# kaiwenShen/Do-You-Really-Need-to-Pay-2-20-Hedge-Fund-Strategy-Replication-via-Machine-Learning

Measured on AMD Instinct MI355X. Metric: seq/sec/node MTSS-WGAN-GP train (24x32 windows) at 1/2/4/8 GPUs; W-dist parity, higher is better.
Workload: dtype fp32; 1 GPU; global_batch=262144, batch_per_gpu=262144, seq_len=24, features=32, parallelism=dp1

## Files before the change

do-you-really-need-to-pay-2-20-hedge-fund-strategy-replication-via-machine-learning_amd/csrc/bindings.cpp:

```cpp
#include <torch/extension.h>
#include <torch/library.h>
#include <ATen/hip/impl/HIPGuardImplMasqueradingAsCUDA.h>
#include <ATen/hip/impl/HIPStreamMasqueradingAsCUDA.h>

#include "kernels.h"
#include "poison.h"

#include <atomic>
#include <cmath>
#include <cstdlib>
#include <cstring>

std::atomic<bool>& hfrep::poison_flag() {
  static std::atomic<bool> f{[] {
    const char* e = getenv("HFREP_POISON");
    return e && e[0] == '1';
  }()};
  return f;
}

namespace {

using at::Tensor;
using c10::optional;
// ... 229 lines not shown
  TORCH_CHECK(dzx.sizes() == gates.sizes(), "lstm_tfwd: shapes");
  const int B = gates.size(0), Tn = gates.size(1), H = gates.size(2) / 4;
  check_lstm_U(U, H);
  GUARD(dzx);
  Tensor hds = out_empty({B, Tn, H}, dzx.options());
  Tensor zds = out_empty_like(gates);
  Tensor cds = out_empty({B, Tn, H}, dzx.options());
  const bool ok = hfrep::launch_lstm_tfwd(dt_of(dzx), dzx.data_ptr(), gates.data_ptr(), cs.data_ptr(),
                                          U.data_ptr<float>(), hds.data_ptr(), zds.data_ptr(), cds.data_ptr(), B, Tn,
                                          H, (int)act, cur_stream(dzx));
  TORCH_CHECK(ok, "lstm_tfwd: hidden size ", H, " not instantiated");
  return {hds, zds, cds};
}

std::tuple<Tensor, Tensor> lstm_tbwd(optional<Tensor> dH, Tensor dHd, Tensor gates, Tensor cs, Tensor zds, Tensor cds,
                                     Tensor U, int64_t act) {
  CHECK_GPU(dHd); CHECK_GPU(gates); CHECK_GPU(cs); CHECK_GPU(zds); CHECK_GPU(cds);
  same_dt(dHd, gates); same_dt(dHd, zds); same_dt(dHd, cds);
  if (dH.has_value()) { CHECK_GPU(*dH); same_dt(*dH, dHd); }
  const int B = gates.size(0), Tn = gates.size(1), H = gates.size(2) / 4;
  check_lstm_U(U, H);
  GUARD(dHd);
  Tensor dZ = out_empty_like(gates), dZd = out_empty_like(gates);
  const bool ok = hfrep::launch_lstm_tbwd(dt_of(dHd), ptr_or_null(dH), dHd.data_ptr(), gates.data_ptr(),
                                          cs.data_ptr(), zds.data_ptr(), cds.data_ptr(), U.data_ptr<float>(),
                                          dZ.data_ptr(), dZd.data_ptr(), B, Tn, H, (int)act, cur_stream(dHd));
  TORCH_CHECK(ok, "lstm_tbwd: hidden size ", H, " not instantiated");
  return {dZ, dZd};
}

bool lstmf_supported(int64_t H, int64_t K, int64_t act) { return hfrep::lstmf_supported((int)H, (int)K, (int)act); }
bool narrowf_supported(int64_t K, int64_t N) { return hfrep::narrowf_supported((int)K, (int)N); }
int64_t set_lstmf_fwd_impl(int64_t v) { return hfrep::set_lstmf_fwd_impl((int)v); }
int64_t set_lstmf_bwd_impl(int64_t v) { return hfrep::set_lstmf_bwd_impl((int)v); }

std::tuple<Tensor, Tensor> lstmf_fwd(Tensor x, Tensor W, optional<Tensor> b, Tensor U, int64_t act, bool save) {
  CHECK_F32(x); CHECK_F32(W);
  TORCH_CHECK(x.dim() == 3, "x must be (B, T, K)");
  const int B = x.size(0), Tn = x.size(1), K = x.size(2), H = U.size(0);
  check_lstm_U(U, H);
  TORCH_CHECK(W.size(0) == K && W.size(1) == 4 * H, "W must be (K, 4H)");
  if (b.has_value()) { CHECK_F32(*b); TORCH_CHECK(b->numel() == 4 * H, "bias size"); }
  TORCH_CHECK(hfrep::lstmf_supported(H, K, (int)act), "lstmf_fwd: unsupported H/K/act");
  GUARD(x);
  Tensor hs = out_empty({B, Tn, H}, x.options());
  Tensor tape = at::empty({save ? (int64_t)hfrep::lstmf_tape_elems(B, Tn) : 0}, x.options());
  const bool ok = hfrep::launch_lstmf_fwd(x.data_ptr<float>(), W.data_ptr<float>(),
                                          b.has_value() ? b->data_ptr<float>() : nullptr, U.data_ptr<float>(),
                                          hs.data_ptr<float>(), save ? tape.data_ptr<float>() : nullptr, B, Tn, K, H,
                                          (int)act, cur_stream(x));
  TORCH_CHECK(ok, "lstmf_fwd: launch failed");
  return {hs, tape};
}

std::tuple<Tensor, Tensor> lstmf_tfwd(Tensor xd, Tensor W, Tensor U, Tensor tape, int64_t act) {
  CHECK_F32(xd); CHECK_F32(W); CHECK_F32(tape);
  TORCH_CHECK(xd.dim() == 3, "xd must be (B, T, K)");
  const int B = xd.size(0), Tn = xd.size(1), K = xd.size(2), H = U.size(0);
  check_lstm_U(U, H);
  TORCH_CHECK(W.size(0) == K && W.size(1) == 4 * H, "W must be (K, 4H)");
  TORCH_CHECK(tape.numel() == (int64_t)hfrep::lstmf_tape_elems(B, Tn), "lstmf_tfwd: tape size");
  TORCH_CHECK(hfrep::lstmf_supported(H, K, (int)act), "lstmf_tfwd: unsupported H/K/act");
  GUARD(xd);
  Tensor hds = out_empty({B, Tn, H}, xd.options());
  Tensor ttape = at::empty_like(tape);
  const bool ok = hfrep::launch_lstmf_tfwd(xd.data_ptr<float>(), W.data_ptr<float>(), U.data_ptr<float>(),
                                           tape.data_ptr<float>(), hds.data_ptr<float>(), ttape.data_ptr<float>(), B, Tn,
                                           K, H, (int)act, cur_stream(xd));
  TORCH_CHECK(ok, "lstmf_tfwd: launch failed");
  return {hds, ttape};
}

static void check_head(const optional<Tensor>& d, const optional<Tensor>& w, const Tensor& like, int64_t B, int64_t n) {
  if (d.has_value()) {
    CHECK_F32(*d);
    TORCH_CHECK(d->numel() == B && d->device() == like.device(), "head adjoint factor: B fp32 values");
  }
  if (w.has_value()) {
    CHECK_F32(*w);
    TORCH_CHECK(w->numel() == n && w->device() == like.device(), "head weight: Tn H fp32 values");
  }
}

Tensor lstmf_bwd(optional<Tensor> dH, Tensor tape, Tensor U, int64_t act, int64_t B, int64_t Tn, optional<Tensor> hd,
                 optional<Tensor> hw) {
  CHECK_F32(tape);
  const int H = U.size(0);
  check_lstm_U(U, H);
  TORCH_CHECK(tape.numel() == (int64_t)hfrep::lstmf_tape_elems(B, Tn), "lstmf_bwd: tape size");
  if (dH.has_value()) { CHECK_F32(*dH); TORCH_CHECK(dH->numel() == B * Tn * H, "lstmf_bwd: dH shape"); }
  TORCH_CHECK(hd.has_value() == hw.has_value() && !(hd.has_value() && dH.has_value()),
              "lstmf_bwd: dH or the head factors (hd, hw)");
  check_head(hd, hw, tape, B, Tn * H);
  GUARD(tape);
  Tensor dZ = out_empty({B, Tn, 4 * H}, tape.options());
  Tensor dHm;
  if (hd.has_value() && !hfrep::lstmf_head_supported()) {
    dHm = out_empty({B, Tn * H}, tape.options());
    hfrep::launch_skinny_dgrad(hfrep::DT_F32, hd->data_ptr<float>(), hw->data_ptr<float>(), dHm.data_ptr(), B,
                               (int)(Tn * H), 1, cur_stream(tape));
  }
  const bool head = hd.has_value() && !dHm.defined();
  const float* dhp = dHm.defined() ? dHm.data_ptr<float>() : dH.has_value() ? dH->data_ptr<float>() : nullptr;
  const bool ok = hfrep::launch_lstmf_bwd(dhp, tape.data_ptr<float>(), U.data_ptr<float>(), dZ.data_ptr<float>(), B, Tn,
                                          H, (int)act, cur_stream(tape), head ? hd->data_ptr<float>() : nullptr,
                                          head ? hw->data_ptr<float>() : nullptr);
  TORCH_CHECK(ok, "lstmf_bwd: unsupported H / act");
  return dZ;
}

std::tuple<Tensor, Tensor> lstmf_tbwd(optional<Tensor> dH, optional<Tensor> dHd, Tensor tape, Tensor ttape, Tensor U,
                                      int64_t act, int64_t B, int64_t Tn, optional<Tensor> hd, optional<Tensor> hdd,
                                      optional<Tensor> hw) {
  CHECK_F32(tape); CHECK_F32(ttape);
  const int H = U.size(0);
  check_lstm_U(U, H);
  TORCH_CHECK(tape.numel() == (int64_t)hfrep::lstmf_tape_elems(B, Tn) && ttape.numel() == tape.numel(), "tape size");
  for (const auto* d : {&dH, &dHd})
    if (d->has_value()) { CHECK_F32(**d); TORCH_CHECK((*d)->numel() == B * Tn * H, "lstmf_tbwd: adjoint shape"); }
  const bool head = hw.has_value();
  TORCH_CHECK(!head || (!dH.has_value() && !dHd.has_value()), "lstmf_tbwd: adjoints (dH, dHd) or head factors, not both");
  check_head(hd, hw, tape, B, Tn * H);
  check_head(hdd, {}, tape, B, Tn * H);
  GUARD(tape);
  Tensor dZ = out_empty({B, Tn, 4 * H}, tape.options()), dZd = out_empty({B, Tn, 4 * H}, tape.options());
  const bool ok = hfrep::launch_lstmf_tbwd(dH.has_value() ? dH->data_ptr<float>() : nullptr,
                                           dHd.has_value() ? dHd->data_ptr<float>() : nullptr, tape.data_ptr<float>(),
                                           ttape.data_ptr<float>(), U.data_ptr<float>(), dZ.data_ptr<float>(),
                                           dZd.data_ptr<float>(), B, Tn, H, (int)act, cur_stream(tape),
                                           head && hd.has_value() ? hd->data_ptr<float>() : nullptr,
                                           head && hdd.has_value() ? hdd->data_ptr<float>() : nullptr,
                                           head ? hw->data_ptr<float>() : nullptr);
  TORCH_CHECK(ok, "lstmf_tbwd: unsupported H / act");
  return {dZ, dZd};
}

Tensor lstmf_dgrad(Tensor dz, Tensor W, int64_t impl) {
  CHECK_F32(dz); CHECK_F32(W);
  TORCH_CHECK(dz.dim() == 2 && dz.is_contiguous() && W.dim() == 2 && W.is_contiguous() && W.size(1) == dz.size(1),
              "lstmf_dgrad: dz (M, N) and W (KO, N), contiguous");
  TORCH_CHECK(hfrep::lstmf_dgrad_supported(dz.size(1), W.size(0)), "lstmf_dgrad: N must be 400 and KO <= 112");
  GUARD(dz);
  Tensor x = out_empty({dz.size(0), W.size(0)}, dz.options());
  if (dz.size(0) == 0) return x;
  const bool ok = hfrep::launch_lstmf_dgrad(dz.data_ptr<float>(), W.data_ptr<float>(), x.data_ptr<float>(), dz.size(0),
                                            dz.size(1), W.size(0), cur_stream(dz), (int)impl);
  TORCH_CHECK(ok, "lstmf_dgrad: launch failed");
  return x;
}

bool is_fp3(const Tensor& t) { return t.scalar_type() == at::kBFloat16 && t.dim() >= 2 && t.size(-2) == 3; }

Tensor fp3_split(Tensor x, bool interleave) {
  CHECK_F32(x);
  TORCH_CHECK(x.is_contiguous() && x.dim() >= 1, "fp3_split: a contiguous fp32 tensor");
  const int64_t C = x.size(-1), M = C ? x.numel() / C : 0;
  auto sz = x.sizes().vec();
  sz.insert(sz.end() - 1, 3);
  GUARD(x);
  Tensor p = out_empty(sz, x.options().dtype(at::kBFloat16));
  hfrep::launch_fp3_split(x.data_ptr<float>(), reinterpret_cast<uint16_t*>(p.data_ptr()), M, (int)C, interleave,
                          cur_stream(x));
  return p;
}

Tensor fp3_join(Tensor p, bool interleave) {
  CHECK_GPU(p);
  TORCH_CHECK(is_fp3(p) && p.is_contiguous(), "fp3_join: contiguous bf16 planes (..., 3, C)");
  const int64_t C = p.size(-1), M = C ? p.numel() / (3 * C) : 0;
  auto sz = p.sizes().vec();
  sz.erase(sz.end() - 2);
  GUARD(p);
  Tensor x = out_empty(sz, p.options().dtype(at::kFloat));
  hfrep::launch_fp3_join(reinterpret_cast<const uint16_t*>(p.data_ptr()), x.data_ptr<float>(), M, (int)C, interleave,
                         cur_stream(p));
  return x;
}

void lstmf_wgrad_p_(Tensor x, Tensor hs, Tensor dZ, Tensor gW, Tensor gU, optional<Tensor> gb, optional<Tensor> xd,
                    optional<Tensor> hds, optional<Tensor> dZd, int64_t impl) {
  CHECK_GPU(x); CHECK_GPU(hs); CHECK_GPU(dZ);
  const int pm = (is_fp3(x) ? 1 : 0) | (is_fp3(hs) ? 2 : 0) | (is_fp3(dZ) ? 4 : 0);
  for (const Tensor* t : {&x, &hs, &dZ})
    TORCH_CHECK(t->is_contiguous() && (is_fp3(*t) ? t->dim() == 4 : (t->scalar_type() == at::kFloat && t->dim() == 3)),
                "lstmf_wgrad_p_: fp32 (B,T,C) or FP3 planes (B,T,3,C), contiguous");
  const int B = x.size(0), Tn = x.size(1), K = x.size(-1), Hd = hs.size(-1), N = dZ.size(-1);
  TORCH_CHECK(hs.size(0) == B && dZ.size(0) == B && hs.size(1) == Tn && dZ.size(1) == Tn, "lstmf_wgrad_p_: B/T");
  TORCH_CHECK(hfrep::lstmf_wgrad_supported(K, Hd, N) && (pm == 0 || K == 32 || K == 100), "lstmf_wgrad_p_: K / H / N");
  CHECK_F32(gW); CHECK_F32(gU);
  TORCH_CHECK(gW.numel() == (int64_t)K * N && gU.numel() == (int64_t)Hd * N, "lstmf_wgrad_p_: grad sizes");
// ... 449 lines not shown
  return out;
}

Tensor p2p_buffer(int64_t cap, int64_t device) {
  TORCH_CHECK(cap > 0, "p2p_buffer: cap must be positive");
  bool fine = false;
  void* p = hfrep::p2p_alloc(cap, (int)device, &fine);
  auto opts = at::TensorOptions().dtype(at::kByte).device(at::Device(at::kCUDA, (int)device));
  return torch::from_blob(p, {(int64_t)hfrep::p2p_buffer_bytes(cap)}, [](void* q) { hfrep::p2p_free(q); }, opts);
}

std::vector<int64_t> p2p_handle(Tensor buf) {
  TORCH_CHECK(buf.is_cuda() && buf.scalar_type() == at::kByte, "p2p_handle: a p2p_buffer tensor");
  uint8_t h[64];
  hfrep::p2p_ipc_handle(buf.data_ptr(), h);
  return std::vector<int64_t>(h, h + 64);
}

int64_t p2p_open(std::vector<int64_t> handle, int64_t device) {
  TORCH_CHECK(handle.size() == 64, "p2p_open: a 64-byte IPC handle");
  uint8_t h[64];
  for (int i = 0; i < 64; ++i) h[i] = (uint8_t)handle[i];
  return (int64_t)reinterpret_cast<intptr_t>(hfrep::p2p_ipc_open(h, (int)device));
}

void p2p_close(int64_t ptr) { hfrep::p2p_ipc_close(reinterpret_cast<void*>((intptr_t)ptr)); }

void p2p_allreduce_(Tensor x, Tensor buf, std::vector<int64_t> peers, int64_t rank, int64_t cap, double scale,
                    double timeout_s) {
  CHECK_F32(x);
  TORCH_CHECK(buf.is_cuda() && buf.scalar_type() == at::kByte && buf.device() == x.device(),
              "p2p_allreduce_: buf must be this device's p2p_buffer");
  const int world = (int)peers.size();
  TORCH_CHECK(world >= 1 && world <= hfrep::kP2PMaxRanks && rank >= 0 && rank < world, "p2p_allreduce_: 1 <= world <= 8");
  TORCH_CHECK(x.numel() <= cap && buf.numel() >= (int64_t)hfrep::p2p_buffer_bytes(cap), "p2p_allreduce_: x exceeds cap");
  TORCH_CHECK(peers[rank] == (int64_t)reinterpret_cast<intptr_t>(buf.data_ptr()), "p2p_allreduce_: peers[rank] must be buf");
  hfrep::P2PPeers pp{};
  for (int r = 0; r < world; ++r) pp.base[r] = reinterpret_cast<char*>((intptr_t)peers[r]);
  TORCH_CHECK(timeout_s > 0, "p2p_allreduce_: timeout_s must be positive");
  GUARD(x);
  static thread_local int s_dev = -1;
  static thread_local double s_sec = -1;
  static thread_local uint64_t s_ticks = 0;
  if (s_dev != x.get_device() || s_sec != timeout_s) {
    s_ticks = hfrep::p2p_timeout_ticks(timeout_s, x.get_device());
    s_dev = x.get_device();
    s_sec = timeout_s;
  }
  hfrep::launch_p2p_allreduce(x.data_ptr<float>(), x.numel(), pp, (int)rank, world, cap, (float)scale, s_ticks,
                              cur_stream(x));
}

int64_t p2p_error(Tensor buf) {
  TORCH_CHECK(buf.is_cuda() && buf.scalar_type() == at::kByte, "p2p_error: a p2p_buffer tensor");
  GUARD(buf);
  return hfrep::p2p_read_error(buf.data_ptr());
}

}

TORCH_LIBRARY(hfrep, m) {
  m.def("linear(Tensor x, Tensor W, Tensor? b, int act, Tensor(a!)? out=None) -> Tensor");
  m.def("linear_dgrad(Tensor dz, Tensor W) -> Tensor");
  m.def("linear_wgrad_(Tensor x, Tensor dz, Tensor(a!) gW, Tensor(b!)? gb, int shiftT=0) -> ()");
  m.def("fp3_split(Tensor x, bool interleave=False) -> Tensor");
  m.def("fp3_join(Tensor p, bool interleave=False) -> Tensor");
  m.def("lstmf_wgrad_p_(Tensor x, Tensor hs, Tensor dZ, Tensor(a!) gW, Tensor(b!) gU, Tensor(c!)? gb, Tensor? xd=None, Tensor? hds=None, Tensor? dZd=None, int impl=0) -> ()");
  m.def("lstmf_dgrad_p(Tensor dzp, Tensor W, int impl=0) -> Tensor");
  m.def("lstm_wgrad_(Tensor x, Tensor hs, Tensor dZ, Tensor(a!) gW, Tensor(b!) gU, Tensor(c!)? gb, Tensor? xd=None, Tensor? hds=None, Tensor? dZd=None, int impl=0) -> ()");
  m.def("act_fwd(Tensor x, int act) -> Tensor");
  m.def("act_bwd(Tensor dy, Tensor y, int act) -> Tensor");
  m.def("act_tangent_bwd(Tensor dyd, Tensor y, Tensor zd, int act) -> Tensor");
  m.def("lstm_fwd(Tensor zx, Tensor U, int act, bool save) -> (Tensor, Tensor, Tensor)");
  m.def("lstm_bwd(Tensor dH, Tensor gates, Tensor cs, Tensor U, int act) -> Tensor");
  m.def("lstm_tfwd(Tensor dzx, Tensor gates, Tensor cs, Tensor U, int act) -> (Tensor, Tensor, Tensor)");
  m.def("lstm_tbwd(Tensor? dH, Tensor dHd, Tensor gates, Tensor cs, Tensor zds, Tensor cds, Tensor U, int act) -> (Tensor, Tensor)");
  m.def("lstmf_supported(int H, int K, int act) -> bool", &lstmf_supported);
  m.def("narrowf_supported(int K, int N) -> bool", &narrowf_supported);
  m.def("set_lstmf_fwd_impl(int v) -> int", &set_lstmf_fwd_impl);
  m.def("set_lstmf_bwd_impl(int v) -> int", &set_lstmf_bwd_impl);
  m.def("lstmf_fwd(Tensor x, Tensor W, Tensor? b, Tensor U, int act, bool save) -> (Tensor, Tensor)");
  m.def("linear_head_cs(Tensor x, Tensor W, Tensor? b, int split, float wa, float wb, Tensor(a!) gW, Tensor(b!)? gb) -> Tensor");
  m.def("linear_head_cs_supported(int K) -> bool", &linear_head_cs_supported);
  m.def("lstmf_bwd(Tensor? dH, Tensor tape, Tensor U, int act, int B, int T, Tensor? hd=None, Tensor? hw=None) -> Tensor");
  m.def("lstmf_tbwd(Tensor? dH, Tensor? dHd, Tensor tape, Tensor ttape, Tensor U, int act, int B, int T, Tensor? hd=None, "
        "Tensor? hdd=None, Tensor? hw=None) -> (Tensor, Tensor)");
  m.def("lstmf_tfwd(Tensor xd, Tensor W, Tensor U, Tensor tape, int act) -> (Tensor, Tensor)");
  m.def("lstmf_dgrad(Tensor dz, Tensor W, int impl=0) -> Tensor");
  m.def("lstm2_fwd(Tensor x, Tensor W, Tensor? b, Tensor U, int act, bool save) -> (Tensor, Tensor)");
  m.def("lstm2_bwd(Tensor? dH, Tensor tape, Tensor U, int act, Tensor? W=None, bool need_dz=True, Tensor? head_d=None, "
        "Tensor? head_w=None) -> (Tensor, Tensor)");
  m.def("lstm2_tfwd(Tensor xd, Tensor W, Tensor U, Tensor tape, int act) -> (Tensor, Tensor)");
  m.def("lstm2_tbwd(Tensor? dH, Tensor? dHd, Tensor tape, Tensor ttape, Tensor U, int act, Tensor? W=None, "
        "Tensor? head_d=None, Tensor? head_dd=None, Tensor? head_w=None) -> (Tensor, Tensor, Tensor, Tensor)");
  m.def("set_debug_poison(bool on) -> bool", &set_debug_poison);
  m.def("layernorm_fwd(Tensor x, Tensor gamma, Tensor beta, float eps, bool save=True, float pre_lrelu=-1.0) -> "
        "(Tensor, Tensor, Tensor)");
  m.def("layernorm_bwd_(Tensor dy, Tensor xhat, Tensor rstd, Tensor gamma, Tensor(a!)? ggamma, Tensor(b!)? gbeta) -> Tensor");
  m.def("layernorm_tfwd(Tensor xd, Tensor xhat, Tensor rstd, Tensor gamma) -> Tensor");
  m.def("layernorm_tbwd_(Tensor? dy, Tensor dyd, Tensor xd, Tensor xhat, Tensor rstd, Tensor gamma, "
        "Tensor(a!) ggamma, Tensor(b!) gbeta, bool need_dx) -> (Tensor, Tensor)");
  m.def("gp_coef(Tensor g, float weight) -> (Tensor, Tensor)");
  m.def("gp_coef_pack(Tensor g, float weight, Tensor w) -> (Tensor, Tensor)");
  m.def("gp_pack(Tensor pen, float weight, Tensor w) -> Tensor");
  m.def("gan_loss(Tensor p, int split, float la, float lb, int kind) -> (Tensor, Tensor)");
  m.def("im2col_causal(Tensor x, int k, int dil) -> Tensor");
  m.def("col2im_causal(Tensor dcols, int k, int dil, int C) -> Tensor");
  m.def("interpolate(Tensor real, Tensor fake, Tensor alpha) -> Tensor");
  m.def("philox_fill_(Tensor(a!) out, int seed, Tensor(b!) ctr, int dist) -> ()");
  m.def("sample_windows(Tensor data, int batch, int seed, Tensor(a!) ctr, ScalarType out_dtype, Tensor(b!)? dst=None) -> Tensor");
  m.def("ae_fit_supported(int A, int k, int batch) -> bool", &ae_fit_supported);
  m.def("ae_fit(Tensor[] Xt, Tensor[] Xv, Tensor[] order, Tensor(a!)[] We, Tensor(b!)[] Wd, Tensor(c!)[] mWe, "
        "Tensor(d!)[] vWe, Tensor(e!)[] mWd, Tensor(f!)[] vWd, Tensor(g!)[] step, Tensor(h!)[] m_cache, int[] patience, "
        "float lr, float b1, float b2, float eps, int batch, bool bf16) -> (Tensor, Tensor)");
  m.def("rmsprop_(Tensor(a!) p, Tensor g, Tensor(b!) ms, float lr, float rho, float eps, float clip, float gscale) -> ()");
  m.def("adam_(Tensor(a!) p, Tensor g, Tensor(b!) m, Tensor(c!) v, Tensor step, float lr, float b1, float b2, float eps, float clip, float gscale) -> ()");
  m.def("nadam_(Tensor(a!) p, Tensor g, Tensor(b!) m, Tensor(c!) v, Tensor step, Tensor m_cache, float lr, float b1, float b2, float eps, float gscale) -> ()");
  m.def("step_advance_(Tensor(a!) step, Tensor(b!)? m_cache, float b1) -> ()");
  m.def("clip_(Tensor(a!) p, float c) -> ()");
  m.def("wdist_sorted(Tensor x, Tensor ref_sorted) -> Tensor");
  m.def("p2p_buffer(int cap, int device) -> Tensor", &p2p_buffer);
  m.def("p2p_handle(Tensor buf) -> int[]");
  m.def("p2p_open(int[] handle, int device) -> int", &p2p_open);
  m.def("p2p_close(int ptr) -> ()", &p2p_close);
  m.def("p2p_allreduce_(Tensor(a!) x, Tensor buf, int[] peers, int rank, int cap, float scale, float timeout_s) -> ()");
  m.def("p2p_error(Tensor buf) -> int");
}

TORCH_LIBRARY_IMPL(hfrep, CUDA, m) {
  m.impl("linear", &linear);
  m.impl("p2p_handle", &p2p_handle);
  m.impl("p2p_allreduce_", &p2p_allreduce_);
  m.impl("p2p_error", &p2p_error);
  m.impl("linear_dgrad", &linear_dgrad);
  m.impl("linear_wgrad_", &linear_wgrad_);
  m.impl("lstm_wgrad_", &lstm_wgrad_);
  m.impl("act_fwd", &act_fwd);
  m.impl("act_bwd", &act_bwd);
  m.impl("act_tangent_bwd", &act_tangent_bwd);
  m.impl("lstm_fwd", &lstm_fwd);
  m.impl("lstmf_fwd", &lstmf_fwd);
  m.impl("lstmf_tfwd", &lstmf_tfwd);
  m.impl("linear_head_cs", &linear_head_cs);
  m.impl("lstmf_bwd", &lstmf_bwd);
  m.impl("lstmf_tbwd", &lstmf_tbwd);
  m.impl("lstmf_dgrad", &lstmf_dgrad);
  m.impl("fp3_split", &fp3_split);
  m.impl("fp3_join", &fp3_join);
  m.impl("lstmf_wgrad_p_", &lstmf_wgrad_p_);
  m.impl("lstmf_dgrad_p", &lstmf_dgrad_p);
  m.impl("lstm_bwd", &lstm_bwd);
  m.impl("lstm_tfwd", &lstm_tfwd);
  m.impl("lstm_tbwd", &lstm_tbwd);
  m.impl("lstm2_fwd", &lstm2_fwd);
  m.impl("lstm2_bwd", &lstm2_bwd);
  m.impl("lstm2_tfwd", &lstm2_tfwd);
  m.impl("lstm2_tbwd", &lstm2_tbwd);
  m.impl("layernorm_fwd", &layernorm_fwd);
  m.impl("layernorm_bwd_", &layernorm_bwd_);
  m.impl("layernorm_tfwd", &layernorm_tfwd);
  m.impl("layernorm_tbwd_", &layernorm_tbwd_);
  m.impl("gp_coef", &gp_coef);
  m.impl("gp_coef_pack", &gp_coef_pack);
  m.impl("gp_pack", &gp_pack);
  m.impl("gan_loss", &gan_loss);
  m.impl("im2col_causal", &im2col_causal);
  m.impl("col2im_causal", &col2im_causal);
  m.impl("interpolate", &interpolate);
  m.impl("philox_fill_", &philox_fill_);
  m.impl("sample_windows", &sample_windows);
  m.impl("ae_fit", &ae_fit);
  m.impl("rmsprop_", &rmsprop_);
  m.impl("adam_", &adam_);
  m.impl("nadam_", &nadam_);
  m.impl("step_advance_", &step_advance_);
  m.impl("clip_", &clip_);
  m.impl("wdist_sorted", &wdist_sorted);
}
```

do-you-really-need-to-pay-2-20-hedge-fund-strategy-replication-via-machine-learning_amd/csrc/kernels.h:

```cpp
#pragma once
#include <hip/hip_runtime.h>
#include <stdint.h>

namespace hfrep {

enum DType : int { DT_F32 = 0, DT_BF16 = 1 };

bool launch_lstm_fwd(int dt, const void* zx, const float* U, void* hs, void* gates, void* cs, int B, int Tn, int H,
                     int act, hipStream_t s);
bool launch_lstm_bwd(int dt, const void* dH, const void* gates, const void* cs, const float* U, void* dZ, int B,
                     int Tn, int H, int act, hipStream_t s);
bool launch_lstm_tfwd(int dt, const void* dzx, const void* gates, const void* cs, const float* U, void* hds,
                      void* zds, void* cds, int B, int Tn, int H, int act, hipStream_t s);
bool launch_lstm_tbwd(int dt, const void* dH, const void* dHd, const void* gates, const void* cs, const void* zds,
                      const void* cds, const float* U, void* dZ, void* dZd, int B, int Tn, int H, int act,
                      hipStream_t s);

size_t lstm2_tape_elems(int B, int Tn);
bool lstm2_supported(int H, int K);
void launch_lstm2_fwd(const void* x, const float* W, const float* b, const float* U, void* hs, void* tape, int B, int Tn,
                      int K, int H, int act, hipStream_t s);
void launch_lstm2_tfwd(const void* xd, const float* W, const float* U, const void* tape, void* hds, void* ttape, int B,
                       int Tn, int K, int H, int act, hipStream_t s);
void launch_lstm2_bwd(const void* dH, const void* tape, const float* U, void* dZ, const float* W, void* dX, int K,
                      int B, int Tn, int H, int act, hipStream_t s, const void* head_d = nullptr,
                      const float* hw = nullptr);
void launch_lstm2_tbwd(const void* dH, const void* dHd, const void* tape, const void* ttape, const float* U, void* dZ,
                       void* dZd, const float* W, void* dX, void* dXd, int K, int B, int Tn, int H, int act,
                       hipStream_t s, const void* head_d = nullptr, const void* head_dd = nullptr,
                       const float* hw = nullptr);

bool lstmf_supported(int H, int K, int act);
size_t lstmf_tape_elems(int B, int Tn);
bool launch_lstmf_fwd(const float* x, const float* W, const float* b, const float* U, float* hs, float* tape, int B,
                      int Tn, int K, int H, int act, hipStream_t s);
bool launch_lstmf_tfwd(const float* xd, const float* W, const float* U, const float* tape, float* hds, float* ttape,
                       int B, int Tn, int K, int H, int act, hipStream_t s);
bool launch_lstmf_bwd(const float* dH, const float* tape, const float* U, float* dZ, int B, int Tn, int H, int act,
                      hipStream_t s, const float* hd = nullptr, const float* hw = nullptr);
bool lstmf_head_supported();
bool launch_lstmf_tbwd(const float* dH, const float* dHd, const float* tape, const float* ttape, const float* U, float* dZ,
                       float* dZd, int B, int Tn, int H, int act, hipStream_t s, const float* hd = nullptr,
                       const float* hdd = nullptr, const float* hw = nullptr);
bool lstmf_wgrad_supported(int K, int H, int N);
size_t lstmf_wgrad_workspace_floats(int M, int K, int impl = 0);
bool launch_lstmf_wgrad(const void* X, const void* Hs, const void* D, const void* Xd, const void* Hds, const void* Dd,
                        float* gW, float* gU, float* gb, int M, int K, int Tn, float* ws, hipStream_t s, int impl = 0,
                        int pm = 0);
bool lstmf_dgrad_supported(int N, int KO);
int set_lstmf_fwd_impl(int v);
int set_lstmf_bwd_impl(int v);
bool launch_lstmf_dgrad(const void* D, const float* W, float* X, int M, int N, int KO, hipStream_t s, int impl = 0,
                        bool pd = false);
void launch_fp3_split(const float* x, uint16_t* p, int64_t M, int C, bool interleave, hipStream_t s);
void launch_fp3_join(const uint16_t* p, float* x, int64_t M, int C, bool interleave, hipStream_t s);

bool ae_fit_supported(int A, int k, int batch);
struct AeFitJob {
  const float* Xt;
  const float* Xv;
  const int* order;
  float *We, *Wd, *mWe, *vWe, *mWd, *vWd, *step, *m_cache;
  double* hist;
  int* nep;
  int nt, nv, epochs, patience, k, pad_;
};
void launch_ae_fit(bool bf16, const AeFitJob* jobs, int njobs, int batch, float lr, float b1, float b2, float eps, int A,
                   hipStream_t s);

void launch_linear(int dt, const void* A, const float* W, const float* bias, void* C, int M, int N, int K,
                   int w_trans, int act, hipStream_t s);
bool fp32_exact_mode();
size_t wgrad_workspace_floats(int M, int K, int N);
void launch_wgrad(int dt, const void* X, const void* D, float* gW, float* gb, int M, int K, int N, int shiftT,
                  float* ws, hipStream_t s);

size_t lstm_wgrad2_workspace_floats(int M, int K, int Hd, int N);
void launch_lstm_wgrad2(const void* X0, const void* H0, const void* D0, const void* X1, const void* H1, const void* D1,
                        float* gW, float* gU, float* gb, int M, int K, int Hd, int N, int Tn, float* ws, hipStream_t s);
void launch_lstm_wgrad2_reduce(const float* ws, float* gW, float* gU, float* gb, int splits, int K, int Hd, int N,
                               hipStream_t s, int Ks = 0);
void launch_linear2(const void* A, const float* W, const float* bias, void* C, int M, int N, int K, int w_trans, int act,
                    hipStream_t s);

bool lstm_wgrad3_supported(int M, int K, int Hd, int N);
size_t lstm_wgrad3_workspace_floats(int K, int Hd, int N);
bool launch_lstm_wgrad3(const void* X0, const void* H0, const void* D0, const void* X1, const void* H1, const void* D1,
                        float* gW, float* gU, float* gb, int M, int K, int Hd, int N, int Tn, float* ws, hipStream_t s);

bool skinny_supported(int K, int N);
bool narrow_supported(int K, int N);
void launch_narrow_fwd(const void* x, const float* W, const float* b, void* y, int M, int K, int N, int act,
                       hipStream_t s);
bool narrowf_supported(int K, int N);
bool widef_supported(int K, int N);
void launch_widef(const float* x, const float* B, int sk, int sn, const float* b, float* y, int M, int K, int N,
                  int act, hipStream_t s);
void launch_narrowf(const float* x, const float* B, int sk, int sn, const float* b, float* y, int M, int K, int N,
                    int act, hipStream_t s);
void launch_skinny_fwd(int dt, const void* x, const float* W, const float* b, void* y, int M, int K, int N, int act,
                       hipStream_t s);
size_t skinny_wgrad_workspace_floats(int M, int K, int N);
void launch_skinny_wgrad(int dt, const void* x, const void* d, float* gW, float* gb, int M, int K, int N, float* ws,
                         hipStream_t s);
void launch_skinny_dgrad(int dt, const void* d, const float* W, void* dx, int M, int K, int N, hipStream_t s);
bool skinny_fwd_cs_supported(int K);
size_t skinny_fwd_cs_workspace_floats(int M, int K);
void launch_skinny_fwd_cs(int dt, const void* x, const float* W, const float* b, void* y, int M, int K, int split,
                          float wa, float wb, float* gW, float* gb, float* ws, hipStream_t s);
void launch_split_reduce(const float* slab, float* a, float* b, int splits, int na, int nb, hipStream_t s);

int device_cu_count();
void launch_im2col_causal(int dt, const void* x, void* cols, int B, int Tn, int C, int k, int dil, hipStream_t s);
void launch_col2im_causal(int dt, const void* dcols, void* dx, int B, int Tn, int C, int k, int dil, hipStream_t s);
void launch_act_fwd(int dt, const void* x, void* y, int64_t n, int act, hipStream_t s);
void launch_act_bwd(int dt, const void* dy, const void* y, void* dx, int64_t n, int act, hipStream_t s);
void launch_act_tangent_bwd(int dt, const void* dyd, const void* y, const void* zd, void* out, int64_t n, int act,
                            hipStream_t s);
void launch_layernorm_fwd(int dt, const void* x, const float* gamma, const float* beta, void* y, void* xhat,
                          float* rstd, int64_t rows, int D, float eps, float pre_alpha, hipStream_t s);
int layernorm_bwd_splits(int64_t rows);
void launch_layernorm_bwd(int dt, const void* dy, const void* xhat, const float* rstd, const float* gamma,
                          void* dx, float* ggamma, float* gbeta, float* ws, int64_t rows, int D, hipStream_t s);
// ... 48 lines not shown
```

do-you-really-need-to-pay-2-20-hedge-fund-strategy-replication-via-machine-learning_amd/csrc/lstm_f32.hip:

```cpp
#include "common.h"
#include "kernels.h"

#include <atomic>
#include <cstdlib>
#include <mutex>
#include <type_traits>
#include <set>
#include <stdexcept>

namespace hfrep {

namespace {

typedef __amdgpu_buffer_rsrc_t rsrc_t;
typedef int v4i_t __attribute__((ext_vector_type(4)));
constexpr int kOOB = 0x7fff0000;

__device__ __forceinline__ rsrc_t make_rsrc(const void* p, int bytes) {
  return __builtin_amdgcn_make_buffer_rsrc(const_cast<void*>(p), 0, bytes, 0x00020000);
}
__device__ __forceinline__ rsrc_t ftile_rsrc(const float* base, int row0, int B, int Tn, int W) {
  row0 = __builtin_amdgcn_readfirstlane(row0);
  const int nr = base ? max(0, min(32, B - row0)) : 0;
  return make_rsrc(base + (nr ? (size_t)row0 * Tn * W : 0), nr * Tn * W * 4);
// ... 633 lines not shown
          const int sd = tt * FH * 4 + 16 * n;
          tg[n] = __builtin_bit_cast(f32x4, __builtin_amdgcn_raw_buffer_load_b128(rt, tok ? tl : kOOB, sg, 0));
          tz[n] = __builtin_bit_cast(f32x4, __builtin_amdgcn_raw_buffer_load_b128(rtt, tok ? tl : kOOB, sg, 0));
          tcp[n] = ld1(rt, (tok && tt > 0) ? tcl : kOOB, sc);
          tcdp[n] = ld1(rtt, (tok && tt > 0) ? tcl : kOOB, sc);
          if constexpr (HEAD) {
            const float wv = ld1(rhw, tok ? hvo : kOOB, sd);
            tdh[n] = hdv[m] * wv;
            tdhd[n] = hddv[m] * wv;
          } else {
            tdh[n] = ld1(rdh, tok ? vp1[m] : kOOB, sd);
            tdhd[n] = ld1(rdhd, tok ? vp1[m] : kOOB, sd);
          }
        }
      };
#pragma unroll
      for (int m = 0; m < 2; ++m)
#pragma unroll
        for (int n = 0; n < FNT; ++n) {
          const bool tok = !(w == 3 && n >= 4);
          const int oc = tcl + (Tn - 1) * FT_STEP * 4 + ftape_slot(m, n);
          acn[m][n] = 0.f;
          acdn[m][n] = 0.f;
          tc[m][n] = ld1(rt, tok ? oc : kOOB, 0);
          tcd[m][n] = ld1(rtt, tok ? oc : kOOB, 0);
        }
      load_half(std::integral_constant<int, 0>{}, Tn - 1, true);
      for (int i = tid; i < 2 * 32 * (BZ_LR + BH_LR); i += 512) zt[i] = 0.f;
      __syncthreads();
      auto half_b = [&](auto M_) {
        constexpr int m = decltype(M_)::value;
#pragma unroll
        for (int n = 0; n < FNT; ++n) {
          const bool tok = !(w == 3 && n >= 4);
          const float i_ = tg[n][0], f_ = tg[n][1], g_ = tg[n][2], o_ = tg[n][3];
          const float zdi = tz[n][0], zdf = tz[n][1], zdg = tz[n][2], zdo = tz[n][3];
          const float c = tc[m][n], cd = tcd[m][n], cp = tcp[n], cdp = tcdp[n];
          const float si = i_ * (1.f - i_), sf = f_ * (1.f - f_), so = o_ * (1.f - o_), sg = act_dy(ACT, g_);
          const float idot = si * zdi, fdot = sf * zdf, gdot = sg * zdg, odot = so * zdo;
          const float ca = act_f(ACT, c), d1 = act_dy(ACT, ca), d2 = act_d2y(ACT, ca);
          const int hi = hr + 16 * m * BH_LR + 4 * n;
          const float a_h = tdh[n] + ht[hi], a_hd = tdhd[n] + hdt[hi];
          const float a_od = a_hd * ca;
          const float a_o = a_h * ca + a_hd * d1 * cd;
          const float a_cd = acdn[m][n] + a_hd * o_ * d1;
          const float a_c = acn[m][n] + a_h * o_ * d1 + a_hd * (odot * d1 + o_ * d2 * cd);
          const float a_fd = a_cd * cp, a_id = a_cd * g_, a_gd = a_cd * i_;
          const float a_f = a_c * cp + a_cd * cdp;
          const float a_i = a_c * g_ + a_cd * gdot;
          const float a_g = a_c * i_ + a_cd * idot;
          acn[m][n] = tok ? a_c * f_ + a_cd * fdot : 0.f;
          acdn[m][n] = tok ? a_cd * f_ : 0.f;
          const float s2i = si * (1.f - 2.f * i_), s2f = sf * (1.f - 2.f * f_), s2o = so * (1.f - 2.f * o_);
          const float s2g = act_d2y(ACT, g_);
          float zd4[4], z4[4];
          zd4[0] = a_id * si; zd4[1] = a_fd * sf; zd4[2] = a_gd * sg; zd4[3] = a_od * so;
          z4[0] = a_i * si + a_id * s2i * zdi;
          z4[1] = a_f * sf + a_fd * s2f * zdf;
          z4[2] = a_g * sg + a_gd * s2g * zdg;
          z4[3] = a_o * so + a_od * s2o * zdo;
          const int zo = zw + 16 * m * BZ_LR + 4 * n;
          float* zp = tok ? zt + zo : trash;
          float* zdp = tok ? zdt + zo : trash;
#pragma unroll
          for (int k = 0; k < 4; ++k) {
            zp[k * BZ_KQ] = z4[k];
            zdp[k * BZ_KQ] = zd4[k];
          }
          tc[m][n] = cp;
          tcd[m][n] = cdp;
          if ((n + 1) % HFREP_TBWD_CELLGROUP == 0 || n == FNT - 1) __builtin_amdgcn_sched_barrier(0);
        }
      };
      using I0 = std::integral_constant<int, 0>;
      using I1 = std::integral_constant<int, 1>;
      for (int t = Tn - 1; t >= 0; --t) {
        half_b(I0{});
        __builtin_amdgcn_sched_barrier(0);
        load_half(I1{}, t, true);
        lds_barrier();
        half_b(I1{});
        __builtin_amdgcn_sched_barrier(0);
        load_half(I0{}, t > 0 ? t - 1 : 0, t > 0);
        lds_barrier();
      }
      __syncthreads();
    }
  }
}

constexpr int WF_R = 16, WF_LA = 272, WF_LD = 400;
template <int KX>
struct WFGeo {
  static constexpr int KR = KX + FH + 1;
  static constexpr int NI = (KR + 15) / 16;
  static_assert(NI <= 16 && 16 * 16 <= WF_LA, "wgrad i tiles");
  static constexpr int NX4 = WF_R * KX / 4, NH4 = WF_R * FH / 4, ND4 = WF_R * FG / 4;
  static constexpr int JX = (NX4 + 511) / 512, JH = (NH4 + 511) / 512, JD = (ND4 + 511) / 512;
};

template <int KX, int XR = KX>
__global__ void __launch_bounds__(512)
lstmf_wgrad_kernel(const float* __restrict__ X, const float* __restrict__ Hs, const float* __restrict__ D,
                   const float* __restrict__ Xd, const float* __restrict__ Hds, const float* __restrict__ Dd,
                   float* __restrict__ slab, int M, int Tn, int rows_per_wg) {
  using WG = WFGeo<KX>;
  constexpr int NI = WG::NI, KR = WG::KR;
  __shared__ __attribute__((aligned(16))) float As[2][WF_R * WF_LA];
  __shared__ __attribute__((aligned(16))) float Ds[2][WF_R * WF_LD];
  __shared__ __attribute__((aligned(16))) float trash4[4];
  const int tid = threadIdx.x, lane = tid & 63;
  const int w = __builtin_amdgcn_readfirstlane(tid >> 6);
  const int g = lane >> 4, c16 = lane & 15;
  const int mb = blockIdx.x * rows_per_wg, me = min(M, mb + rows_per_wg);
  for (int i = tid; i < 2 * WF_R * WF_LA; i += 512) (&As[0][0])[i] = 0.f;

  f32x4 acc[NI][3], accx[2];
#pragma unroll
  for (int it = 0; it < NI; ++it)
#pragma unroll
    for (int jj = 0; jj < 3; ++jj) acc[it][jj] = f32x4{0.f, 0.f, 0.f, 0.f};
  accx[0] = accx[1] = f32x4{0.f, 0.f, 0.f, 0.f};
  const int ie0 = min(2 * w, 15), ie1 = min(2 * w + 1, 15);

  f32x4 vx[WG::JX], vh[WG::JH], vd[WG::JD];
  for (int seg = 0; seg < (Xd ? 2 : 1); ++seg) {
    const float* Xs = seg ? Xd : X;
    const float* Hq = seg ? Hds : Hs;
    const float* Dq = seg ? Dd : D;
    const int hb = mb > 0 ? mb - 1 : 0, nr = me > mb ? me - mb : 0;
    const rsrc_t rx = make_rsrc(Xs + (size_t)mb * XR, nr * XR * 4);
    const rsrc_t rh = make_rsrc(Hq + (size_t)hb * FH, (nr ? me - hb : 0) * FH * 4);
    const rsrc_t rd = make_rsrc(Dq + (size_t)mb * FG, nr * FG * 4);
    auto load = [&](int m0) {
#pragma unroll
      for (int j = 0; j < WG::JX; ++j) {
        const int e = tid + 512 * j, r = e / (KX / 4), c = e - r * (KX / 4);
        const bool ok = e < WG::NX4 && m0 + r < me;
        vx[j] = ldx4<XR>(rx, ok ? ((m0 - mb + r) * XR + 4 * c) * 4 : kOOB, 0, 4 * c);
      }
#pragma unroll
      for (int j = 0; j < WG::JH; ++j) {
        const int e = tid + 512 * j, r = e / (FH / 4), c = e - r * (FH / 4);
        const int m = m0 + r;
        const bool ok = e < WG::NH4 && m < me && (m % Tn) != 0;
        vh[j] = __builtin_bit_cast(f32x4, __builtin_amdgcn_raw_buffer_load_b128(rh, ok ? ((m - 1 - hb) * FH + 4 * c) * 4 : kOOB, 0, 0));
      }
#pragma unroll
      for (int j = 0; j < WG::JD; ++j) {
        const int e = tid + 512 * j, r = e / (FG / 4), c = e - r * (FG / 4);
        const bool ok = e < WG::ND4 && m0 + r < me;
        vd[j] = __builtin_bit_cast(f32x4, __builtin_amdgcn_raw_buffer_load_b128(rd, ok ? ((m0 - mb + r) * FG + 4 * c) * 4 : kOOB, 0, 0));
      }
    };
    auto to_lds = [&](int buf) {
#pragma unroll
      for (int j = 0; j < WG::JX; ++j) {
        const int e = tid + 512 * j, r = e / (KX / 4), c = e - r * (KX / 4);
        *reinterpret_cast<f32x4*>(e < WG::NX4 ? &As[buf][r * WF_LA + 4 * c] : trash4) = vx[j];
      }
#pragma unroll
      for (int j = 0; j < WG::JH; ++j) {
        const int e = tid + 512 * j, r = e / (FH / 4), c = e - r * (FH / 4);
        *reinterpret_cast<f32x4*>(e < WG::NH4 ? &As[buf][r * WF_LA + KX + 4 * c] : trash4) = vh[j];
      }
#pragma unroll
// ... 806 lines not shown
            t6 = mma32(a0, up[ks][n][2], t6);
            t6 = mma32(a1, up[ks][n][1], t6);
            t6 = mma32(a1, up[ks][n][0], t6);
            t6 = mma32(a0, up[ks][n][1], t6);
            acc[n] = mma32(a0, up[ks][n][0], t6);
          }
          __builtin_amdgcn_sched_barrier(0);
        }
        {
          const float at = *reinterpret_cast<const __attribute__((address_space(3))) float*>(hcur + aht + 16 * m * 16);
#pragma unroll
          for (int n = 0; n < FNT; ++n) acc[n] = mma4(at, ut[n], acc[n]);
        }
#pragma unroll
        for (int n = 0; n < FNT; ++n) {
          const bool tok = !(w == 3 && n >= 4);
          const int v1 = tok ? p1 + 16 * n : kOOB;
          const f32x4 zs = acc[n];
          float hv;
          if constexpr (!TAN) {
            float y[4];
#pragma unroll
            for (int i = 0; i < 4; ++i) {
              const float s_ = zs[i] + bq[n];
              const float e = am * __builtin_amdgcn_rcpf(1.f + __builtin_amdgcn_exp2f(s_)) + bm;
              y[i] = glin ? s_ : e;
            }
            quad_transpose(y, q);
            const float cn = y[1] * cst[m][n] + y[0] * y[2];
            float ca;
            if constexpr (ACT == ACT_TANH) ca = 2.f * __builtin_amdgcn_rcpf(1.f + __builtin_amdgcn_exp2f(GSC * cn)) - 1.f;
            else if constexpr (ACT == ACT_SIGMOID) ca = __builtin_amdgcn_rcpf(1.f + __builtin_amdgcn_exp2f(GSC * cn));
            else ca = cn;
            hv = tok ? y[3] * ca : 0.f;
            cst[m][n] = cn;
            if constexpr (TAPE) {
              st4(f32x4{y[0], y[1], y[2], y[3]}, rt, tok ? tl + tb + ftape_slot(m, n) : kOOB);
              st1(cn, rt, tok ? tcl + tb + ftape_slot(m, n) : kOOB, 0);
            }
          } else {
            float zd[4] = {zs[0], zs[1], zs[2], zs[3]};
            quad_transpose(zd, q);
            const f32x4 y = pg[n];
            const float idot = y[0] * (1.f - y[0]) * zd[0], fdot = y[1] * (1.f - y[1]) * zd[1];
            const float gdot = act_dy(ACT, y[2]) * zd[2], odot = y[3] * (1.f - y[3]) * zd[3];
            const float c = pc[n];
            float cdn = fdot * cprev[m][n] + y[1] * cst[m][n] + idot * y[2] + y[0] * gdot;
            const float ca = act_f(ACT, c);
            float hd = odot * ca + y[3] * act_dy(ACT, ca) * cdn;
            if (!tok) { cdn = 0.f; hd = 0.f; }
            cst[m][n] = cdn;
            cprev[m][n] = c;
            hv = hd;
            st4(f32x4{zd[0], zd[1], zd[2], zd[3]}, rt, tok ? tl + tb + ftape_slot(m, n) : kOOB);
            st1(cdn, rt, tok ? tcl + tb + ftape_slot(m, n) : kOOB, 0);
          }
          {
            const int u = ub + 4 * n, row = 16 * m + 4 * g + q;
            const uint32_t h1 = trunc_hi(hv);
            const float r1 = hv - __builtin_bit_cast(float, h1);
            const uint32_t m1 = trunc_hi(r1);
            const uint32_t l1 = __builtin_bit_cast(uint32_t, r1 - __builtin_bit_cast(float, m1));
            const bool pl = u < 96;
            lds_char* dp = pl ? hnext + (row * FS_HR + u) * 2 : trashc;
            *reinterpret_cast<__attribute__((address_space(3))) uint16_t*>(dp) = (uint16_t)(h1 >> 16);
            *reinterpret_cast<__attribute__((address_space(3))) uint16_t*>(dp + (pl ? FS_HPL : 0)) = (uint16_t)(m1 >> 16);
            *reinterpret_cast<__attribute__((address_space(3))) uint16_t*>(dp + (pl ? 2 * FS_HPL : 0)) = (uint16_t)(l1 >> 16);
            const bool tl4 = u >= 96 && u < FH;
            lds_char* tp = tl4 ? hnext + 3 * FS_HPL + (row * 4 + (u - 96)) * 4 : trashc;
            *reinterpret_cast<__attribute__((address_space(3))) float*>(tp) = hv;
          }
          st1(hv, rh, v1, 0);
        }
      }
      xp.to_lds(xb + ((t + 1) & 1) * 32 * GX::LR, trash);
      lds_barrier();
    }
  }
}

constexpr int BS_LZ = 432;
constexpr int BS_PL = 32 * BS_LZ * 2;

template <int ACT, bool HEAD = false>
__global__ void __launch_bounds__(256, 1)
lstmf_bwds_kernel(const float* __restrict__ dH, const float* __restrict__ tape, const float* __restrict__ U,
                  float* __restrict__ dZ, int B, int Tn, const float* __restrict__ hd, const float* __restrict__ hw) {
  extern __shared__ __attribute__((aligned(16))) float fsm[];
  float* zt = fsm;
  float* ht = zt + 32 * BZ_LR;
  float* trash = ht + 32 * BH_LR;
  lds_char* trashp = (lds_char*)(trash + 4 * BZ_KQ);
  lds_char* zp = (lds_char*)(trash + 4 * BZ_KQ + 4);
  const int tid = threadIdx.x, lane = tid & 63;
  const int w = __builtin_amdgcn_readfirstlane(tid >> 6);
  const int q = lane & 3, g = lane >> 4, j4 = (lane & 15) >> 2, c16 = lane & 15;
  const int nrb = (B + 31) / 32;
  bf16x8 up[2][DS_KS][3];
#pragma unroll
  for (int e = 0; e < 2; ++e) {
    const int col = 16 * (2 * w + e) + c16;
    const bool ok = col < FH;
#pragma unroll
    for (int ks = 0; ks < DS_KS; ++ks) {
      f32x4 v[2];
#pragma unroll
      for (int j = 0; j < 8; ++j) {
        const int k = min(32 * ks + 8 * g + j, FG - 1);
        const float x = U[(ok ? col : 0) * FG + (k & 3) * FH + (k >> 2)];
        v[j >> 2][j & 3] = (ok && 32 * ks + 8 * g + j < FG) ? x : 0.f;
      }
      uint32_t p0[3][2], p1[3][2];
      split3(v[0], p0);
      split3(v[1], p1);
#pragma unroll
      for (int p = 0; p < 3; ++p) {
        up[e][ks][p] = __builtin_bit_cast(bf16x8, make_uint4(p0[p][0], p0[p][1], p1[p][0], p1[p][1]));
        if (e == 1 || ks < 8) asm volatile("" : "+a"(up[e][ks][p]));
      }
    }
  }
  const int ub = FUW * w + j4;
  const int hr = (4 * g + q) * BH_LR + ub, zw = (4 * g + q) * BZ_LR + ub;
  const int zpw = ((4 * g + q) * BS_LZ + 4 * ub) * 2;
  const int ao = (c16 * BS_LZ + 8 * g) * 2;
  const int srr = tid / 100, sch = tid - 100 * srr, sqq = sch / 25, sc = sch - 25 * sqq;
  const int slo = (srr & 1) * BZ_LR + sqq * BZ_KQ + 4 * sc;
  const int sgo = tid < 200 ? (srr * Tn * FG + sqq * FH + 4 * sc) * 4 : kOOB;
  const int tl = ftape_lane(w, lane), tcl = ftape_cell(w, lane);
  using I0 = std::integral_constant<int, 0>;
  using I1 = std::integral_constant<int, 1>;
  for (int rb = blockIdx.x; rb < nrb; rb += gridDim.x) {
    const int row0 = rb * 32;
    const rsrc_t rdh = ftile_rsrc(dH, row0, B, Tn, FH), rt = ftape_rsrc(tape, rb, nrb, Tn);
    const rsrc_t rz = ftile_rsrc(dZ, row0, B, Tn, FG);
    const int nr = min(32, B - row0);
    int vp1[2];
#pragma unroll
    for (int m = 0; m < 2; ++m) vp1[m] = ((16 * m + 4 * g + q) * Tn * FH + ub) * 4;
    float hdv[2] = {0.f, 0.f};
    const rsrc_t rhw = make_rsrc(hw, HEAD ? Tn * FH * 4 : 0);
    if constexpr (HEAD) {
#pragma unroll
      for (int m = 0; m < 2; ++m) {
        const int r = row0 + 16 * m + 4 * g + q;
        hdv[m] = r < B ? hd[r] : 0.f;
      }
    }
    const int hvo = ub * 4;
    float dc[2][FNT], tc[2][FNT];
    f32x4 tg[FNT];
    float tcp[FNT], tdh[FNT];
    const int T1 = Tn - 1;
#pragma unroll
    for (int n = 0; n < FNT; ++n) {
      const bool tok = !(w == 3 && n >= 4);
#pragma unroll
      for (int m = 0; m < 2; ++m) {
        dc[m][n] = 0.f;
        tc[m][n] = ld1(rt, tok ? tcl + T1 * FT_STEP * 4 + ftape_slot(m, n) : kOOB, 0);
      }
      bwdf_tape_load_u<HEAD>(tg[n], tcp[n], tdh[n], rt, rdh, tl, tcl, vp1[0], T1 * FT_STEP * 4 + ftape_slot(0, n),
                             max(T1 - 1, 0) * FT_STEP * 4 + ftape_slot(0, n), T1 * FH * 4 + 16 * n, tok, T1 > 0, hdv[0],
                             rhw, hvo);
    }
    for (int i = tid; i < 3 * BS_PL / 16; i += 256)
      reinterpret_cast<__attribute__((address_space(3))) u32x4_t*>(zp)[i] = u32x4_t{0, 0, 0, 0};
    for (int i = tid; i < 32 * BH_LR; i += 256) ht[i] = 0.f;
    __syncthreads();
    auto store_half = [&](auto M_, int ts) {
      constexpr int M = decltype(M_)::value;
#pragma unroll
      for (int k = 8 * M; k < 8 * M + 8; ++k) {
        const f32x4 v = *reinterpret_cast<const f32x4*>(zt + slo + 2 * k * BZ_LR);
        st16(v, rz, 2 * k + srr < nr, sgo, (2 * k * Tn + ts) * FG * 4);
      }
    };
    auto cell = [&](auto M_, int n, float hrec, int t) {
      constexpr int m = decltype(M_)::value;
      const bool tok = !(w == 3 && n >= 4);
      const float ig = tg[n][0], fg = tg[n][1], gg = tg[n][2], og = tg[n][3];
      const float dht = tdh[n] + hrec;
      const float ca = act_f(ACT, tc[m][n]);
      const float dov = dht * ca;
      const float dct = dc[m][n] + dht * og * act_dy(ACT, ca);
      dc[m][n] = tok ? dct * fg : 0.f;
      f32x4 z4;
      z4[0] = dct * gg * ig * (1.f - ig);
      z4[1] = dct * tcp[n] * fg * (1.f - fg);
      z4[2] = dct * ig * act_dy(ACT, gg);
      z4[3] = dov * og * (1.f - og);
      float* zd = tok ? zt + zw + 16 * m * BZ_LR + 4 * n : trash;
#pragma unroll
      for (int k = 0; k < 4; ++k) zd[k * BZ_KQ] = z4[k];
      uint32_t p[3][2];
      split3(z4, p);
      lds_char* pd = tok ? zp + zpw + 16 * m * BS_LZ * 2 + 32 * n : trashp;
      const int ps = tok ? BS_PL : 0;
#pragma unroll
      for (int pp = 0; pp < 3; ++pp)
        *reinterpret_cast<__attribute__((address_space(3))) u32x2_t*>(pd + pp * ps) = u32x2_t{p[pp][0], p[pp][1]};
      tc[m][n] = tcp[n];
      if constexpr (m == 0) {
        bwdf_tape_load_u<HEAD>(tg[n], tcp[n], tdh[n], rt, rdh, tl, tcl, vp1[1], t * FT_STEP * 4 + ftape_slot(1, n),
                               max(t - 1, 0) * FT_STEP * 4 + ftape_slot(1, n), t * FH * 4 + 16 * n, tok, t > 0, hdv[1],
                               rhw, hvo);
      } else {
        const int tp = t > 0 ? t - 1 : 0;
        bwdf_tape_load_u<HEAD>(tg[n], tcp[n], tdh[n], rt, rdh, tl, tcl, vp1[0], tp * FT_STEP * 4 + ftape_slot(0, n),
                               max(tp - 1, 0) * FT_STEP * 4 + ftape_slot(0, n), tp * FH * 4 + 16 * n, tok && t > 0,
                               tp > 0, hdv[0], rhw, hvo);
      }
    };
    auto phase = [&](auto MA_, int t) {
      constexpr int MA = decltype(MA_)::value;
      if constexpr (MA == 1) {
        if (t < T1) store_half(I1{}, t + 1);
      } else {
        store_half(I0{}, t);
      }
      float hv[FNT];
#pragma unroll
      for (int n = 0; n < FNT; ++n) hv[n] = ht[hr + 16 * (1 - MA) * BH_LR + 4 * n];
      __builtin_amdgcn_sched_barrier(0);
      f32x4 acc[2] = {f32x4{0.f, 0.f, 0.f, 0.f}, f32x4{0.f, 0.f, 0.f, 0.f}};
      const lds_char* ar = zp + ao + 16 * MA * BS_LZ * 2;
      bf16x8 af[2][3];
#pragma unroll
      for (int p = 0; p < 3; ++p) af[0][p] = *reinterpret_cast<const __attribute__((address_space(3))) bf16x8*>(ar + p * BS_PL);
#pragma unroll
      for (int ks = 0; ks < DS_KS; ++ks) {
        if (ks + 1 < DS_KS) {
#pragma unroll
          for (int p = 0; p < 3; ++p)
            af[(ks + 1) & 1][p] = *reinterpret_cast<const __attribute__((address_space(3))) bf16x8*>(ar + p * BS_PL + 64 * (ks + 1));
        }
        const bf16x8(&a)[3] = af[ks & 1];
#pragma unroll
        for (int e = 0; e < 2; ++e) {
          acc[e] = mma32(a[2], up[e][ks][0], acc[e]);
          acc[e] = mma32(a[0], up[e][ks][2], acc[e]);
          acc[e] = mma32(a[1], up[e][ks][1], acc[e]);
          acc[e] = mma32(a[1], up[e][ks][0], acc[e]);
          acc[e] = mma32(a[0], up[e][ks][1], acc[e]);
          acc[e] = mma32(a[0], up[e][ks][0], acc[e]);
        }
        if (ks < FNT) cell(std::integral_constant<int, 1 - MA>{}, ks, hv[ks], t);
      }
#pragma unroll
      for (int ks = 0; ks < DS_KS; ++ks) {
        __builtin_amdgcn_sched_group_barrier(0x100, 3, 0);
#pragma unroll
        for (int i = 0; i < 12; ++i) {
          __builtin_amdgcn_sched_group_barrier(0x008, 1, 0);
          __builtin_amdgcn_sched_group_barrier(0x002, 3, 0);
        }
      }
      __builtin_amdgcn_sched_barrier(0);
#pragma unroll
      for (int e = 0; e < 2; ++e) {
        const bool ok = 2 * w + e < 7;
        float* hd = ok ? ht + (16 * MA + 4 * g) * BH_LR + 16 * (2 * w + e) + c16 : trash;
        const int hs = ok ? BH_LR : 0;
#pragma unroll
        for (int i = 0; i < 4; ++i) hd[i * hs] = acc[e][i];
      }
      lds_barrier();
    };
    for (int t = T1; t >= 0; --t) {
      phase(I1{}, t);
      phase(I0{}, t);
    }
    store_half(I1{}, 0);
    __syncthreads();
  }
}

constexpr int DS4_RS = 432;
constexpr int DS4_PL = 16 * DS4_RS * 2;
constexpr int DS4_BUF = 3 * DS4_PL;
constexpr int DS4_SLOTS = (16 * 100 + 255) / 256;
constexpr int DS4_K0 = DS_KS - DS4_SLOTS;
constexpr int DS4_NS = 2;

template <int NT2, bool PD = false>
__global__ void __launch_bounds__(256, 1)
lstmf_dgrad_s4_kernel(const void* __restrict__ D, const float* __restrict__ W, float* __restrict__ X, int M, int KO) {
  constexpr int DRB = PD ? 6 * FG : 4 * FG;
  extern __shared__ __attribute__((aligned(16))) char dsm_[];
  lds_char* dsm = (lds_char*)dsm_;
  const int tid = threadIdx.x, lane = tid & 63;
  const int w = __builtin_amdgcn_readfirstlane(tid >> 6);
  const int g = lane >> 4, c16 = lane & 15;
  const int nch = (M + 15) / 16;
  bf16x8 bw[2][DS_KS][3];
// ... 227 lines not shown

void allow_lds(const void* k) {
  static std::mutex mu;
  static std::set<const void*> done;
  std::lock_guard<std::mutex> gd(mu);
  if (done.insert(k).second)
    HFREP_CHECK_HIP(hipFuncSetAttribute(k, hipFuncAttributeMaxDynamicSharedMemorySize, (int)F_LDS_MAX));
}
template <int KX>
constexpr size_t fwds_smem() {
  return (size_t)(2 * 32 * FGeo<KX>::LR) * 4 + 2 * FS_HB + 16;
}
static bool fp32_exact() {
  return fp32_exact_mode();
}
static std::atomic<int>& fwdf_impl() {
  static std::atomic<int> v{fp32_exact() ? 1 : 2};
  return v;
}
static int fwdf_version() { return fwdf_impl().load(std::memory_order_relaxed); }
template <int ACT, int KX, bool TAPE, bool TAN>
void fwdf_launch(const float* x, const float* W, const float* b, const float* U, const float* pt, float* hs, float* tp,
                 int B, int Tn, hipStream_t s) {
  const int nrb = (B + 31) / 32, cus = device_cu_count();
  if constexpr (FGeo<KX>::KS <= 8 || (FGeo<KX>::KS <= 12 && !TAN)) {
    if (fwdf_version() == 2) {
      auto k = lstmf_fwds_kernel<ACT, KX, TAPE, TAN>;
      allow_lds(reinterpret_cast<const void*>(k));
      hipLaunchKernelGGL(k, dim3(nrb < cus ? nrb : cus), dim3(256), fwds_smem<KX>(), s, x, W, b, U, pt, hs, tp, B, Tn);
      return;
    }
  }
  auto k = lstmf_fwd_kernel<ACT, KX, TAPE, TAN>;
  allow_lds(reinterpret_cast<const void*>(k));
  hipLaunchKernelGGL(k, dim3(nrb < cus ? nrb : cus), dim3(256), fwdf_smem<KX>(), s, x, W, b, U, pt, hs, tp, B, Tn);
}
template <int KX, bool TAPE, bool TAN>
void fwdf_act(int act, const float* x, const float* W, const float* b, const float* U, const float* pt, float* hs,
              float* tp, int B, int Tn, hipStream_t s) {
  switch (act) {
    case ACT_LINEAR: fwdf_launch<ACT_LINEAR, KX, TAPE, TAN>(x, W, b, U, pt, hs, tp, B, Tn, s); break;
    case ACT_SIGMOID: fwdf_launch<ACT_SIGMOID, KX, TAPE, TAN>(x, W, b, U, pt, hs, tp, B, Tn, s); break;
    default: fwdf_launch<ACT_TANH, KX, TAPE, TAN>(x, W, b, U, pt, hs, tp, B, Tn, s); break;
  }
}
template <bool TAPE, bool TAN>
bool fwdf_k(int K, int act, const float* x, const float* W, const float* b, const float* U, const float* pt, float* hs,
            float* tp, int B, int Tn, hipStream_t s) {
  switch (K) {
    case 32: fwdf_act<32, TAPE, TAN>(act, x, W, b, U, pt, hs, tp, B, Tn, s); return true;
    case 35: fwdf_act<35, TAPE, TAN>(act, x, W, b, U, pt, hs, tp, B, Tn, s); return true;
    case 36: fwdf_act<36, TAPE, TAN>(act, x, W, b, U, pt, hs, tp, B, Tn, s); return true;
    case 100: fwdf_act<100, TAPE, TAN>(act, x, W, b, U, pt, hs, tp, B, Tn, s); return true;
    default: return false;
  }
}
}

int set_lstmf_fwd_impl(int v) { return fwdf_impl().exchange(v); }

bool lstmf_supported(int H, int K, int act) {
  return H == FH && (K == 32 || K == 35 || K == 36 || K == 100) && (act == ACT_LINEAR || act == ACT_SIGMOID || act == ACT_TANH);
}

bool launch_lstmf_fwd(const float* x, const float* W, const float* b, const float* U, float* hs, float* tape, int B,
                      int Tn, int K, int H, int act, hipStream_t s) {
  if (!lstmf_supported(H, K, act) || B <= 0 || Tn <= 0) return false;
  if (tape) return fwdf_k<true, false>(K, act, x, W, b, U, nullptr, hs, tape, B, Tn, s);
  return fwdf_k<false, false>(K, act, x, W, b, U, nullptr, hs, nullptr, B, Tn, s);
}

bool launch_lstmf_tfwd(const float* xd, const float* W, const float* U, const float* tape, float* hds, float* ttape,
                       int B, int Tn, int K, int H, int act, hipStream_t s) {
  if (!lstmf_supported(H, K, act) || B <= 0 || Tn <= 0) return false;
  return fwdf_k<true, true>(K, act, xd, W, nullptr, U, tape, hds, ttape, B, Tn, s);
}

static std::atomic<int>& bwdf_impl() {
  static std::atomic<int> v{fp32_exact() ? 2 : 3};
  return v;
}
template <int ACT>
void bwdf_launch(const float* dH, const float* tape, const float* U, float* dZ, int B, int Tn, hipStream_t s,
                 const float* hd, const float* hw) {
  const int ver = bwdf_impl().load(std::memory_order_relaxed);
  const int nrb = (B + 31) / 32, cus = device_cu_count();
  const size_t sm = (size_t)(32 * BZ_LR + 32 * BH_LR + 4 * BZ_KQ) * 4;
  if (ver != 2) {
    auto go = [&](auto k) {
      allow_lds(reinterpret_cast<const void*>(k));
      hipLaunchKernelGGL(k, dim3(nrb < cus ? nrb : cus), dim3(256), sm + 16 + 3 * BS_PL, s, dH, tape, U, dZ, B, Tn, hd,
                         hw);
    };
    if (hd) go(lstmf_bwds_kernel<ACT, true>);
    else go(lstmf_bwds_kernel<ACT, false>);
    return;
  }
  if (hd) throw std::runtime_error("lstmf_bwd: the exact-fp32 BPTT takes a materialised dH (lstmf_head_supported)");
  auto k = lstmf_bwdp_kernel<ACT>;
  allow_lds(reinterpret_cast<const void*>(k));
  hipLaunchKernelGGL(k, dim3(nrb < cus ? nrb : cus), dim3(512), sm, s, dH, tape, U, dZ, B, Tn);
}
static_assert((32 * BZ_LR + 32 * BH_LR + 4 * BZ_KQ) * 4 + 16 + 3 * BS_PL <= F_LDS_MAX, "split BPTT LDS");
int set_lstmf_bwd_impl(int v) { return bwdf_impl().exchange(v); }
bool lstmf_head_supported() { return bwdf_impl().load(std::memory_order_relaxed) != 2; }
bool launch_lstmf_bwd(const float* dH, const float* tape, const float* U, float* dZ, int B, int Tn, int H, int act,
                      hipStream_t s, const float* hd, const float* hw) {
  if (H != FH || B <= 0 || Tn <= 0) return false;
  switch (act) {
    case ACT_LINEAR: bwdf_launch<ACT_LINEAR>(dH, tape, U, dZ, B, Tn, s, hd, hw); return true;
    case ACT_SIGMOID: bwdf_launch<ACT_SIGMOID>(dH, tape, U, dZ, B, Tn, s, hd, hw); return true;
    case ACT_TANH: bwdf_launch<ACT_TANH>(dH, tape, U, dZ, B, Tn, s, hd, hw); return true;
    default: return false;
  }
}

template <int ACT>
void tbwdf_launch(const float* dH, const float* dHd, const float* tape, const float* ttape, const float* U, float* dZ,
                  float* dZd, int B, int Tn, hipStream_t s, const float* hd, const float* hdd, const float* hw) {
  const int cus = device_cu_count();
  const size_t sm = (size_t)(2 * 32 * BZ_LR + 2 * 32 * BH_LR + 4 * BZ_KQ) * 4;
  const int nrb = (B + 31) / 32;
  auto go = [&](auto k) {
    allow_lds(reinterpret_cast<const void*>(k));
    hipLaunchKernelGGL(k, dim3(nrb < cus ? nrb : cus), dim3(512), sm, s, dH, dHd, tape, ttape, U, dZ, dZd, B, Tn, hd, hdd,
                       hw);
  };
  if (hw) go(lstmf_tbwdp_kernel<ACT, true>);
  else go(lstmf_tbwdp_kernel<ACT, false>);
}
bool launch_lstmf_tbwd(const float* dH, const float* dHd, const float* tape, const float* ttape, const float* U, float* dZ,
                       float* dZd, int B, int Tn, int H, int act, hipStream_t s, const float* hd, const float* hdd,
                       const float* hw) {
  if (H != FH || B <= 0 || Tn <= 0) return false;
  switch (act) {
    case ACT_LINEAR: tbwdf_launch<ACT_LINEAR>(dH, dHd, tape, ttape, U, dZ, dZd, B, Tn, s, hd, hdd, hw); return true;
    case ACT_SIGMOID: tbwdf_launch<ACT_SIGMOID>(dH, dHd, tape, ttape, U, dZ, dZd, B, Tn, s, hd, hdd, hw); return true;
    case ACT_TANH: tbwdf_launch<ACT_TANH>(dH, dHd, tape, ttape, U, dZ, dZd, B, Tn, s, hd, hdd, hw); return true;
    default: return false;
  }
}
size_t lstmf_tape_elems(int B, int Tn) { return (size_t)((B + 31) / 32) * Tn * FT_STEP; }

static int wgradf_grid(int M) {
  const int chunks = (M + WF_R - 1) / WF_R, cus = device_cu_count();
  return chunks < cus ? chunks : cus;
}
bool lstmf_wgrad_supported(int K, int H, int N) { return H == FH && N == FG && (K == 32 || K == 35 || K == 36 || K == 100); }

static int wgradf_version() { return fp32_exact() ? 1 : 0; }
static int wgrads_z(int M) {
  const int chunks = (M + 31) / 32, half = device_cu_count() / 2;
  return chunks < half ? chunks : half;
}
static int wgradq_z(int M) {
  const int chunks = (M + 31) / 32, q = device_cu_count() / 4;
  return chunks < q ? chunks : q;
}
static int wgradf_pick(int impl, int K, int M) {
  (void)M;
  int v = impl >= 1 && impl <= 3 ? impl : wgradf_version();
  if (K == 35 && v == 3) v = 2;
  return v ? v : (K <= 36 ? 2 : 3);
}
size_t lstmf_wgrad_workspace_floats(int M, int K, int impl) {
  const int v = wgradf_pick(impl, K, M);
  const int z = v == 1 ? wgradf_grid(M) : v == 3 ? wgradq_z(M) : wgrads_z(M);
  return (size_t)z * ((K == 35 ? 36 : K) + FH + 1) * FG;
}

bool launch_lstmf_wgrad(const void* X, const void* Hs, const void* D, const void* Xd, const void* Hds, const void* Dd,
                        float* gW, float* gU, float* gb, int M, int K, int Tn, float* ws, hipStream_t s, int impl, int pm) {
  if (!lstmf_wgrad_supported(K, FH, FG) || M <= 0) return false;
  if (pm != 0 && (wgradf_pick(impl, K, M) == 1 || K == 35 || K == 36))
    throw std::runtime_error("lstmf_wgrad: FP3-plane operands need the split kernels and K in {32, 100}");
  if (wgradf_pick(impl, K, M) == 3) {
    const int z0 = wgradq_z(M);
    const int rpz = ((M + z0 - 1) / z0 + 31) / 32 * 32;
    const int z = (M + rpz - 1) / rpz;
    auto go = [&](auto k, size_t sm) {
      allow_lds(reinterpret_cast<const void*>(k));
      hipLaunchKernelGGL(k, dim3(4 * z), dim3(512), sm, s, X, Hs, D, Xd, Hds, Dd, ws, M, Tn, rpz, z);
    };
    switch (K * 8 + pm) {
#define HFREP_Q4(KK, PP) case KK * 8 + PP: go(lstmf_wgrad_q4_kernel<KK, PP>, 2 * WQGeo<KK>::Img::BUF); break;
      HFREP_Q4(32, 0) HFREP_Q4(36, 0) HFREP_Q4(100, 0)
      HFREP_Q4(32, 4) HFREP_Q4(32, 6) HFREP_Q4(32, 7) HFREP_Q4(100, 4) HFREP_Q4(100, 6) HFREP_Q4(100, 7)
#undef HFREP_Q4
      default: throw std::runtime_error("lstmf_wgrad: no quad kernel for this K / plane mask");
    }
    launch_lstm_wgrad2_reduce(ws, gW, gU, gb, z, K, FH, FG, s);
    return true;
  }
  if (wgradf_pick(impl, K, M) != 1) {
    const int z0 = wgrads_z(M);
    const int rpz = ((M + z0 - 1) / z0 + 31) / 32 * 32;
    const int z = (M + rpz - 1) / rpz;
    auto go = [&](auto k, size_t sm) {
      allow_lds(reinterpret_cast<const void*>(k));
      hipLaunchKernelGGL(k, dim3(2 * z), dim3(512), sm, s, X, Hs, D, Xd, Hds, Dd, ws, M, Tn, rpz, z);
    };
    switch (K * 8 + pm) {
      case 35 * 8: go(lstmf_wgrad_split_kernel<36, 35>, 2 * WSGeo<36>::Img::BUF); break;
      case 36 * 8: go(lstmf_wgrad_split_kernel<36>, 2 * WSGeo<36>::Img::BUF); break;
      case 100 * 8: go(lstmf_wgrad_split_kernel<100>, 2 * WSGeo<100>::Img::BUF); break;
#define HFREP_WS(PP) case 32 * 8 + PP: go(lstmf_wgrad_split_kernel<32, 32, PP>, 2 * WSGeo<32>::Img::BUF); break;
      HFREP_WS(0) HFREP_WS(4) HFREP_WS(6) HFREP_WS(7)
#undef HFREP_WS
      default: throw std::runtime_error("lstmf_wgrad: no pair kernel for this K / plane mask");
    }
    launch_lstm_wgrad2_reduce(ws, gW, gU, gb, z, K, FH, FG, s, K == 35 ? 36 : K);
    return true;
  }
  const int grid = wgradf_grid(M);
  const int rpw = ((M + grid - 1) / grid + WF_R - 1) / WF_R * WF_R;
  const int z = (M + rpw - 1) / rpw;
  const float *Xf = static_cast<const float*>(X), *Hf = static_cast<const float*>(Hs), *Df = static_cast<const float*>(D);
  const float *Xdf = static_cast<const float*>(Xd), *Hdf = static_cast<const float*>(Hds), *Ddf = static_cast<const float*>(Dd);
  switch (K) {
    case 32: hipLaunchKernelGGL(lstmf_wgrad_kernel<32>, dim3(z), dim3(512), 0, s, Xf, Hf, Df, Xdf, Hdf, Ddf, ws, M, Tn, rpw); break;
    case 35: hipLaunchKernelGGL((lstmf_wgrad_kernel<36, 35>), dim3(z), dim3(512), 0, s, Xf, Hf, Df, Xdf, Hdf, Ddf, ws, M, Tn, rpw); break;
// ... 72 lines not shown
```

do-you-really-need-to-pay-2-20-hedge-fund-strategy-replication-via-machine-learning_amd/models/layers.py:

```python
from __future__ import annotations

import math
from dataclasses import dataclass

import numpy as np
import torch

from ..ops import functional as Fn
from ..ops import reference as R


def glorot_uniform(shape, gen, fan_in=None, fan_out=None):
    if fan_in is None:
        fan_in, fan_out = shape[0], shape[-1]
    lim = math.sqrt(6.0 / (fan_in + fan_out))
    return (torch.rand(shape, generator=gen, dtype=torch.float64) * 2 - 1) * lim


def orthogonal(shape, gen, gain=1.0):
    rows = int(np.prod(shape[:-1]))
    cols = shape[-1]
    a = torch.randn(max(rows, cols), min(rows, cols), generator=gen, dtype=torch.float64)
    q, r = torch.linalg.qr(a)
    q = q * torch.sign(torch.diagonal(r))
    if rows < cols:
        q = q.t()
    return (gain * q).reshape(shape)


@dataclass
class ParamSpec:
    name: str
    shape: tuple
    init: str
    keras: str = ""
    offset: int = 0


class Layer:

    kind = "layer"
    index = 0

    def __init__(self):
        self.model = None
        self.specs: list[ParamSpec] = []
        self.name = ""

    def build(self, in_shape):
        raise NotImplementedError

    def p(self, name):
        return self.model.view(self, name)

    def g(self, name):
        return self.model.gview(self, name)

    def forward(self, x):
        raise NotImplementedError

    def efwd(self, x, save: bool):
        raise NotImplementedError

    def ebwd(self, ctx, dy, need_dx: bool, wgrad: bool = True):
        raise NotImplementedError

    def etfwd(self, ctx, xd):
        raise NotImplementedError

    def etbwd(self, ctx, tctx, dy, dyd, need_dx: bool):
        raise NotImplementedError

    def w(self, name):
        return self.p(name)


class Dense(Layer):
    kind = "dense"

    def __init__(self, units: int, activation=None, use_bias: bool = True):
        super().__init__()
        self.units, self.act, self.use_bias = units, activation, use_bias
        self.act_code = R.act_code(activation)

    def build(self, in_shape):
        fin = in_shape[-1]
        self.specs = [ParamSpec("kernel", (fin, self.units), "glorot")]
        if self.use_bias:
            self.specs.append(ParamSpec("bias", (self.units,), "zeros"))
        return tuple(in_shape[:-1]) + (self.units,)

    def forward(self, x):
        return R.dense(x, self.w("kernel"), self.w("bias") if self.use_bias else None, self.act)

    def efwd(self, x, save, out=None, compute=True, wgrad_rows=None):
        if not compute:
            assert self.act_code == 0, "only a linear Dense output can be left uncomputed"
            y = torch.empty(tuple(x.shape[:-1]) + (self.units,), dtype=x.dtype, device=x.device)
            return y, ({"x": x, "y": y} if save else None)
        b = self.p("bias") if self.use_bias else None
        if (wgrad_rows is not None and save and out is None and self.units == 1 and self.act_code == 0
                and Fn.head_cs_ok(x, self.p("kernel"))):
            split, wa, wb = wgrad_rows
            y = Fn.linear_head_cs(x, self.p("kernel"), b, split, wa, wb, self.g("kernel"),
                                  self.g("bias") if self.use_bias else None)
            return y, {"x": x, "y": y, "wgrad_done": True}
        y = Fn.linear(x, self.p("kernel"), b, self.act_code, out=out)
        return y, ({"x": x, "y": y} if save else None)

    def _dgrad(self, dz):
        if self.units == 1 and dz.dim() == 2 and Fn.outer_adjoint_ok(dz):
            return Fn.OuterAdjoint(dz, self.p("kernel"))
        return Fn.linear_dgrad(dz, self.p("kernel"))

    def ebwd(self, ctx, dy, need_dx, wgrad=True):
        dz = Fn.act_backward(dy, ctx["y"], self.act_code)
        if wgrad and not ctx.get("wgrad_done"):
            Fn.run_wgrad(Fn.linear_wgrad_, ctx["x"], dz, self.g("kernel"), self.g("bias") if self.use_bias else None)
        return self._dgrad(dz) if need_dx else None

    def etfwd(self, ctx, xd, compute=True):
        if not compute:
            assert self.act_code == 0, "only a linear Dense output can be left uncomputed"
            zd = torch.empty(tuple(xd.shape[:-1]) + (self.units,), dtype=xd.dtype, device=xd.device)
            return zd, {"xd": xd, "zd": zd}
        zd = Fn.linear(xd, self.p("kernel"), None, 0)
        yd = Fn.act_backward(zd, ctx["y"], self.act_code)
        return yd, {"xd": xd, "zd": zd}

    def etbwd(self, ctx, tctx, dy, dyd, need_dx):
        dzd = Fn.act_backward(dyd, ctx["y"], self.act_code)
        zero_dz = dy is None and self.act_code in (0, 3, 4)
        if not zero_dz:
            dz = Fn.act_tangent_backward(dy, dyd, ctx["y"], tctx["zd"], self.act_code)
            Fn.run_wgrad(Fn.linear_wgrad_, ctx["x"], dz, self.g("kernel"), self.g("bias") if self.use_bias else None)
        Fn.run_wgrad(Fn.linear_wgrad_, tctx["xd"], dzd, self.g("kernel"), None)
        if not need_dx:
            return None, None
        return (None if zero_dz else self._dgrad(dz)), self._dgrad(dzd)


class LSTM(Layer):
    kind = "lstm"
    accepts_outer = True

    def __init__(self, units: int, activation="tanh", return_sequences: bool = True):
        super().__init__()
        assert return_sequences, "the reference uses return_sequences=True everywhere"
        self.units, self.act = units, activation
        self.act_code = R.act_code(activation)

    def build(self, in_shape):
        fin = in_shape[-1]
        H = self.units
        self.specs = [
            ParamSpec("kernel", (fin, 4 * H), "glorot"),
            ParamSpec("recurrent_kernel", (H, 4 * H), "orthogonal"),
            ParamSpec("bias", (4 * H,), "lstm_bias"),
        ]
        return tuple(in_shape[:-1]) + (H,)

    def forward(self, x):
        return R.lstm(x, self.w("kernel"), self.w("recurrent_kernel"), self.w("bias"), act=self.act)

    def efwd(self, x, save):
        hs, tape = Fn.lstm_layer_fwd(x, self.p("kernel"), self.p("bias"), self.p("recurrent_kernel"), self.act_code,
                                     save)
        return hs, ({"x": x, "hs": hs, "tape": tape} if save else None)

    def ebwd(self, ctx, dy, need_dx, wgrad=True):
        U = self.p("recurrent_kernel")
        dx = None
        if need_dx:
            dZ, dx = Fn.lstm_layer_bwd(dy, ctx["tape"], U, self.act_code, W=self.p("kernel"), need_dz=wgrad)
        else:
            dZ = Fn.lstm_layer_bwd(dy, ctx["tape"], U, self.act_code)
        if wgrad:
            Fn.run_wgrad(Fn.lstm_wgrad_, ctx["x"], ctx["hs"], dZ, self.g("kernel"), self.g("recurrent_kernel"), self.g("bias"))
        return dx

    def etfwd(self, ctx, xd):
        hds, ttape = Fn.lstm_layer_tfwd(xd, self.p("kernel"), ctx["tape"], self.p("recurrent_kernel"), self.act_code)
        return hds, {"xd": xd, "hds": hds, "ttape": ttape}

    def etbwd(self, ctx, tctx, dy, dyd, need_dx):
        U = self.p("recurrent_kernel")
        dx = dxd = None
        if need_dx:
            dZ, dZd, dx, dxd = Fn.lstm_layer_tbwd(dy, dyd, ctx["tape"], tctx["ttape"], U, self.act_code,
                                                  W=self.p("kernel"))
        else:
            dZ, dZd = Fn.lstm_layer_tbwd(dy, dyd, ctx["tape"], tctx["ttape"], U, self.act_code)
        Fn.run_wgrad(Fn.lstm_wgrad_, ctx["x"], ctx["hs"], dZ, self.g("kernel"), self.g("recurrent_kernel"), self.g("bias"),
                       tctx["xd"], tctx["hds"], dZd)
        return dx, dxd


class LayerNormalization(Layer):
    kind = "layer_normalization"

    def __init__(self, epsilon: float = R.LN_EPS):
        super().__init__()
        self.eps = epsilon

    def build(self, in_shape):
        d = in_shape[-1]
        self.specs = [ParamSpec("gamma", (d,), "ones"), ParamSpec("beta", (d,), "zeros")]
        return tuple(in_shape)

    def forward(self, x):
        return R.layer_norm(x, self.w("gamma"), self.w("beta"), self.eps)

    def efwd(self, x, save):
        y, xhat, rstd = Fn.layer_norm_fwd(x, self.p("gamma"), self.p("beta"), self.eps, save=save)
        return y, ({"x": x, "xhat": xhat, "rstd": rstd} if save else None)

    def ebwd(self, ctx, dy, need_dx, wgrad=True):
        gg, gb = (self.g("gamma"), self.g("beta")) if wgrad else (None, None)
        dx = Fn.layer_norm_bwd_(dy, ctx["xhat"], ctx["rstd"], self.p("gamma"), gg, gb)
        return dx if need_dx else None

    def etfwd(self, ctx, xd):
        return Fn.layer_norm_tfwd(xd, ctx["xhat"], ctx["rstd"], self.p("gamma")), {"xd": xd}

    def etbwd(self, ctx, tctx, dy, dyd, need_dx):
        return Fn.layer_norm_tbwd_(dy, dyd, tctx["xd"], ctx["xhat"], ctx["rstd"], self.p("gamma"), self.g("gamma"),
                                   self.g("beta"), need_dx)


class LeakyReLU(Layer):
    kind = "leaky_re_lu"

    def __init__(self, alpha: float = R.LRELU_ALPHA):
        super().__init__()
        self.alpha = alpha

    def build(self, in_shape):
        return tuple(in_shape)

    def forward(self, x):
        return R.leaky_relu(x, self.alpha)

    def efwd(self, x, save):
        y = Fn.act_forward(x, 3)
        return y, ({"y": y} if save else None)

    def ebwd(self, ctx, dy, need_dx, wgrad=True):
        return Fn.act_backward(dy, ctx["y"], 3) if need_dx else None

    def etfwd(self, ctx, xd):
        return Fn.act_backward(xd, ctx["y"], 3), {}

    def etbwd(self, ctx, tctx, dy, dyd, need_dx):
        if not need_dx:
            return None, None
        dx = Fn.act_backward(dy, ctx["y"], 3) if dy is not None else None
        return dx, Fn.act_backward(dyd, ctx["y"], 3)


class Flatten(Layer):
    kind = "flatten"
    accepts_outer = True

    def build(self, in_shape):
        self.in_shape = tuple(in_shape)
        return (int(np.prod(in_shape)),)

    def forward(self, x):
        return x.reshape(x.shape[0], -1)

    def efwd(self, x, save):
        return x.reshape(x.shape[0], -1), ({"shape": x.shape} if save else None)

    def ebwd(self, ctx, dy, need_dx, wgrad=True):
        return dy.reshape(ctx["shape"]) if need_dx else None

    def etfwd(self, ctx, xd):
        return xd.reshape(xd.shape[0], -1), {}

    def etbwd(self, ctx, tctx, dy, dyd, need_dx):
        if not need_dx:
            return None, None
        return (dy.reshape(ctx["shape"]) if dy is not None else None), dyd.reshape(ctx["shape"])


class Conv1D(Layer):

    kind = "conv1d"

    def __init__(self, filters: int, kernel_size: int, activation=None, dilation: int = 1):
        super().__init__()
        self.filters, self.k, self.act, self.dil = filters, kernel_size, activation, dilation
        self.act_code = R.act_code(activation)

    def build(self, in_shape):
        T, cin = in_shape[-2], in_shape[-1]
        self.cin = cin
        self.specs = [ParamSpec("kernel", (self.k, cin, self.filters), "glorot_conv"),
                      ParamSpec("bias", (self.filters,), "zeros")]
        return (T, self.filters)

    def forward(self, x):
        return R.conv1d_causal(x, self.w("kernel"), self.w("bias"), self.act, self.dil)

    def _unfold(self, x):
        return Fn.im2col_causal(x, self.k, self.dil)

    def efwd(self, x, save):
        cols = self._unfold(x)
        y = Fn.linear(cols, self.p("kernel").reshape(-1, self.filters), self.p("bias"), self.act_code)
        return y, ({"x": x, "cols": cols, "y": y} if save else None)

    def ebwd(self, ctx, dy, need_dx, wgrad=True):
        dz = Fn.act_backward(dy, ctx["y"], self.act_code)
        if wgrad:
            Fn.run_wgrad(Fn.linear_wgrad_, ctx["cols"], dz, self.g("kernel").reshape(-1, self.filters), self.g("bias"))
        if not need_dx:
            return None
        dcols = Fn.linear_dgrad(dz, self.p("kernel").reshape(-1, self.filters))
        return Fn.col2im_causal(dcols, self.k, self.dil, self.cin)

    def etfwd(self, ctx, xd):
        cols_d = self._unfold(xd)
        zd = Fn.linear(cols_d, self.p("kernel").reshape(-1, self.filters), None, 0)
        return Fn.act_backward(zd, ctx["y"], self.act_code), {"cols_d": cols_d, "zd": zd}

    def etbwd(self, ctx, tctx, dy, dyd, need_dx):
        Wk = self.p("kernel").reshape(-1, self.filters)
        gk = self.g("kernel").reshape(-1, self.filters)
        if dy is None:
            dy = torch.zeros_like(ctx["y"])
        dzd = Fn.act_backward(dyd, ctx["y"], self.act_code)
        dz = Fn.act_tangent_backward(dy, dyd, ctx["y"], tctx["zd"], self.act_code)
        Fn.run_wgrad(Fn.linear_wgrad_, ctx["cols"], dz, gk, self.g("bias"))
        Fn.run_wgrad(Fn.linear_wgrad_, tctx["cols_d"], dzd, gk, None)
        if not need_dx:
            return None, None
        return (Fn.col2im_causal(Fn.linear_dgrad(dz, Wk), self.k, self.dil, self.cin),
                Fn.col2im_causal(Fn.linear_dgrad(dzd, Wk), self.k, self.dil, self.cin))


def _init_tensor(spec: ParamSpec, gen, layer: Layer) -> torch.Tensor:
    if spec.init == "glorot":
        return glorot_uniform(spec.shape, gen)
    if spec.init == "glorot_conv":
        k, cin, cout = spec.shape
        return glorot_uniform(spec.shape, gen, fan_in=k * cin, fan_out=k * cout)
    if spec.init == "orthogonal":
        return orthogonal(spec.shape, gen)
    if spec.init == "zeros":
        return torch.zeros(spec.shape, dtype=torch.float64)
    if spec.init == "ones":
        return torch.ones(spec.shape, dtype=torch.float64)
    if spec.init == "lstm_bias":
        H = spec.shape[0] // 4
        b = torch.zeros(spec.shape, dtype=torch.float64)
        b[H:2 * H] = 1.0
        return b
    raise ValueError(spec.init)


_ALIGN = 64


class Sequential(torch.nn.Module):

    _name_counters: dict = {}

    def __init__(self, layers: list[Layer], input_shape, name: str = "sequential", seed: int | None = None,
                 device="cpu", dtype=torch.float32, keras_names: bool = True):
        super().__init__()
        self.layers = list(layers)
        self.input_shape = tuple(input_shape)
        self.model_name = name
        shape = self.input_shape
        off = 0
        self._index: dict = {}
        for li, layer in enumerate(self.layers):
            layer.model = self
            cnt = Sequential._name_counters.get(layer.kind, 0) + 1 if keras_names else li + 1
            Sequential._name_counters[layer.kind] = cnt
            sfx = "" if cnt == 1 else f"_{cnt - 1}"
            layer.name = f"{layer.kind}{sfx}"
            layer.in_shape_, shape = shape, layer.build(shape)
            layer.out_shape_ = shape
            for s in layer.specs:
                n = int(np.prod(s.shape))
                s.offset = off
                cell = f"{layer.name}/lstm_cell{sfx}/" if layer.kind == "lstm" else f"{layer.name}/"
                s.keras = f"{cell}{s.name}:0"
                self._index[(id(layer), s.name)] = s
                off += (n + _ALIGN - 1) // _ALIGN * _ALIGN
        self.output_shape = shape
        self.numel_padded = max(off, _ALIGN)
        gen = torch.Generator().manual_seed(seed if seed is not None else 123)
        flat = torch.zeros(self.numel_padded, dtype=torch.float64)
        for layer in self.layers:
            for s in layer.specs:
                n = int(np.prod(s.shape))
                flat[s.offset:s.offset + n] = _init_tensor(s, gen, layer).reshape(-1)
        self.flat = torch.nn.Parameter(flat.to(dtype=dtype, device=device))
        self.flat.grad = torch.zeros_like(self.flat)
        self.compute_dtype = dtype

    def spec(self, layer, name) -> ParamSpec:
        return self._index[(id(layer), name)]

    def view(self, layer, name):
        s = self.spec(layer, name)
        n = int(np.prod(s.shape))
        return self.flat[s.offset:s.offset + n].view(s.shape)

    def gview(self, layer, name):
        s = self.spec(layer, name)
        n = int(np.prod(s.shape))
        return self.flat.grad[s.offset:s.offset + n].view(s.shape)

    def named_weights(self):
        return [(s.keras, self.view(l, s.name)) for l in self.layers for s in l.specs]

    def get_weights(self):
        return [v.detach().cpu().numpy().copy() for _, v in self.named_weights()]

    def set_weights(self, arrays):
        with torch.no_grad():
            for (_, v), a in zip(self.named_weights(), arrays):
                v.copy_(torch.as_tensor(np.asarray(a), dtype=v.dtype).reshape(v.shape))

    def count_params(self) -> int:
        return sum(int(np.prod(s.shape)) for l in self.layers for s in l.specs)

    def zero_grad(self, set_to_none: bool = False):
        self.flat.grad.zero_()

    def to(self, *args, **kwargs):
        super().to(*args, **kwargs)
        if self.flat.grad is None or self.flat.grad.shape != self.flat.shape or self.flat.grad.device != self.flat.device:
            self.flat.grad = torch.zeros_like(self.flat)
        return self

    def summary(self) -> str:
        lines = [f'Model: "{self.model_name}"', f"{'Layer':<28}{'Output':<20}{'Params':>10}"]
        for l in self.layers:
            n = sum(int(np.prod(s.shape)) for s in l.specs)
            lines.append(f"{l.name:<28}{str((None,) + tuple(l.out_shape_)):<20}{n:>10}")
        lines.append(f"Total params: {self.count_params()}")
        return "\n".join(lines)

    def forward(self, x):
        for l in self.layers:
            x = l.forward(x)
        return x

    def _head_skippable(self) -> bool:
        last = self.layers[-1] if self.layers else None
        return isinstance(last, Dense) and last.act_code == 0

    def efwd(self, x, save: bool = True, out=None, head_out: bool = True, head_wgrad=None):
        skip_head = not head_out and self._head_skippable()
        tape = []
        i, n = 0, len(self.layers)
        while i < n:
            l = self.layers[i]
            if isinstance(l, LeakyReLU) and i + 1 < n and isinstance(self.layers[i + 1], LayerNormalization):
                ln = self.layers[i + 1]
                y, xhat, rstd = Fn.lrelu_layer_norm_fwd(x, ln.p("gamma"), ln.p("beta"), ln.eps, l.alpha, save)
                tape.append({"y": x} if save else None)
                tape.append({"x": None, "x_pre": x, "alpha": l.alpha, "xhat": xhat, "rstd": rstd} if save else None)
                x = y
                i += 2
                continue
            if skip_head and i == n - 1:
                x, ctx = l.efwd(x, save, compute=False)
            elif head_wgrad is not None and i == n - 1 and isinstance(l, Dense) and out is None:
                x, ctx = l.efwd(x, save, wgrad_rows=head_wgrad)
            elif out is not None and i == n - 1 and isinstance(l, Dense):
                x, ctx = l.efwd(x, save, out=out)
            else:
                x, ctx = l.efwd(x, save)
            tape.append(ctx)
            i += 1
        if out is not None and x.data_ptr() != out.data_ptr():
            x = out.copy_(x)
        return x, tape

    @torch.no_grad()
    def predict(self, x, out=None):
        return self.efwd(x, save=False, out=out)[0]

    @staticmethod
    def _adj(layer, dy):
        if isinstance(dy, Fn.OuterAdjoint) and not getattr(layer, "accepts_outer", False):
            return dy.materialize()
        return dy

    def ebwd(self, tape, dy, need_dx: bool = False, wgrad: bool = True, hook=None):
        for i in range(len(self.layers) - 1, -1, -1):
            need = need_dx or i > 0
            layer = self.layers[i]
            dy = layer.ebwd(tape[i], self._adj(layer, dy), need, wgrad)
            if hook is not None:
                hook(i)
        return Fn._mat(dy)

    def etfwd(self, tape, xd, head_out: bool = True):
        skip_head = not head_out and self._head_skippable()
        ttape = []
        n = len(self.layers)
        for i, (l, ctx) in enumerate(zip(self.layers, tape)):
            if skip_head and i == n - 1:
                xd, tctx = l.etfwd(ctx, xd, compute=False)
            else:
                xd, tctx = l.etfwd(ctx, xd)
            ttape.append(tctx)
        return xd, ttape

    def etbwd(self, tape, ttape, dy, dyd, need_dx: bool = False, hook=None):
        for i in range(len(self.layers) - 1, -1, -1):
            need = need_dx or i > 0
            layer = self.layers[i]
            dy, dyd = layer.etbwd(tape[i], ttape[i], self._adj(layer, dy), self._adj(layer, dyd), need)
            if hook is not None:
                hook(i)
        return Fn._mat(dy), Fn._mat(dyd)

    def grad_buckets(self, n: int = 2) -> list[tuple[int, int, int]]:
        starts = []
        for li, l in enumerate(self.layers):
            if l.specs:
                starts.append((li, min(s.offset for s in l.specs)))
        if not starts:
            return []
        total = self.numel_padded
        cuts = [starts[0]]
        for k in range(1, max(n, 1)):
            goal = total * k / n
            li, off = min(starts[1:] or starts, key=lambda c: abs(c[1] - goal))
            if off > cuts[-1][1]:
                cuts.append((li, off))
        out = []
        for j, (li, off) in enumerate(cuts):
            end = cuts[j + 1][1] if j + 1 < len(cuts) else total
            out.append((li, off, end))
        return out[::-1]
```

do-you-really-need-to-pay-2-20-hedge-fund-strategy-replication-via-machine-learning_amd/ops/functional.py:

```python
from __future__ import annotations

import contextlib

import torch

from . import _native
from . import reference as R


def _nat(t: torch.Tensor) -> bool:
    return _native.use_native_for(t)


def _ops():
    return _native.native()


def _2d(x: torch.Tensor) -> torch.Tensor:
    return x.reshape(-1, x.shape[-1])


class _WgradDefer:
    stream = None
    keep: list = []
# ... 240 lines not shown
    return a * real + (1 - a) * fake


def _use_lstm2(x: torch.Tensor, U: torch.Tensor) -> bool:
    return (x.dtype == torch.bfloat16 and U.shape[0] == 100 and x.shape[-1] <= 128 and _nat(x)
            and not _native.fallback_allowed())


def _lstm2_dx_fused(W) -> bool:
    return W is not None and W.shape[0] <= 112


def _use_lstmf(x: torch.Tensor, U: torch.Tensor, act: int) -> bool:
    return (x.dtype == torch.float32 and _nat(x) and not _native.fallback_allowed()
            and bool(_ops().lstmf_supported(int(U.shape[0]), int(x.shape[-1]), int(act))))


class FTape:

    __slots__ = ("t", "B", "T")

    def __init__(self, t: torch.Tensor, B: int, T: int):
        self.t, self.B, self.T = t, int(B), int(T)


def lstm_layer_fwd(x, W, b, U, act: int, save: bool):
    if _use_lstm2(x, U):
        hs, tape = _ops().lstm2_fwd(x.contiguous(), W, b, U, int(act), bool(save))
        return hs, (tape if save else None)
    if _use_lstmf(x, U, act):
        hs, tape = _ops().lstmf_fwd(x.contiguous(), W, b, U, int(act), bool(save))
        return hs, (FTape(tape, x.shape[0], x.shape[1]) if save else None)
    zx = linear(x, W, b, 0)
    hs, gates, cs = lstm_seq_fwd(zx, U, act, save)
    return hs, ((gates, cs) if save else None)


class OuterAdjoint:

    def __init__(self, d: torch.Tensor, w: torch.Tensor, shape=None):
        self.d, self.w = d, w
        self.shape = tuple(shape) if shape is not None else (d.shape[0], w.shape[0])

    def reshape(self, *shape):
        shape = tuple(shape[0]) if len(shape) == 1 and not isinstance(shape[0], int) else tuple(shape)
        return OuterAdjoint(self.d, self.w, shape)

    def materialize(self) -> torch.Tensor:
        return linear_dgrad(self.d, self.w).reshape(self.shape)


def outer_adjoint_ok(dz: torch.Tensor) -> bool:
    return dz.dtype in (torch.bfloat16, torch.float32) and _nat(dz) and not _native.fallback_allowed()


def _mat(a):
    return a.materialize() if isinstance(a, OuterAdjoint) else a


def lstm_layer_bwd(dH, tape, U, act: int, W=None, need_dz: bool = True):
    if isinstance(tape, FTape):
        if isinstance(dH, OuterAdjoint) and dH.d.dtype == torch.float32:
            dZ = _ops().lstmf_bwd(None, tape.t, U, int(act), tape.B, tape.T, dH.d.contiguous(),
                                  dH.w.reshape(-1).contiguous())
        else:
            dH = _mat(dH)
            dZ = _ops().lstmf_bwd(None if dH is None else dH.contiguous(), tape.t, U, int(act), tape.B, tape.T)
        return dZ if W is None else (dZ, linear_dgrad(dZ, W))
    if isinstance(tape, torch.Tensor):
        Wk = W if _lstm2_dx_fused(W) else None
        nd = bool(need_dz or Wk is None)
        if isinstance(dH, OuterAdjoint):
            dZ, dX = _ops().lstm2_bwd(None, tape, U, int(act), Wk, nd, dH.d.contiguous(), dH.w.reshape(-1).contiguous())
        else:
            dZ, dX = _ops().lstm2_bwd(dH.contiguous(), tape, U, int(act), Wk, nd)
        if W is not None and Wk is None:
            dX = linear_dgrad(dZ, W)
        if W is not None and not need_dz:
            dZ = None
        return dZ if W is None else (dZ, dX)
    dH = _mat(dH)
    gates, cs = tape
    dZ = lstm_seq_bwd(dH, gates, cs, U, act)
    return dZ if W is None else (dZ, linear_dgrad(dZ, W))


def lstm_layer_tfwd(xd, W, tape, U, act: int):
    if isinstance(tape, FTape):
        hds, ttape = _ops().lstmf_tfwd(xd.contiguous(), W, U, tape.t, int(act))
        return hds, FTape(ttape, tape.B, tape.T)
    if isinstance(tape, torch.Tensor):
        hds, ttape = _ops().lstm2_tfwd(xd.contiguous(), W, U, tape, int(act))
        return hds, ttape
    gates, cs = tape
    dzx = linear(xd, W, None, 0)
    hds, zds, cds = lstm_seq_tfwd(dzx, gates, cs, U, act)
    return hds, (zds, cds)


def lstm_wgrad_(x, hs, dZ, gW, gU, gb, xd=None, hds=None, dZd=None, impl: int = 0) -> None:
    f32 = (dZ.dtype == torch.float32 and x.shape[-1] in (32, 35, 36, 100) and hs.shape[-1] == 100
           and dZ.shape[-1] == 400)
    if (dZ.dtype == torch.bfloat16 or f32) and _nat(dZ):
        _ops().lstm_wgrad_(x.contiguous(), hs.contiguous(), dZ.contiguous(), gW, gU, gb,
                           None if xd is None else xd.contiguous(), None if hds is None else hds.contiguous(),
                           None if dZd is None else dZd.contiguous(), int(impl))
        return
    T = hs.shape[1]
    linear_wgrad_(x, dZ, gW, gb)
    linear_wgrad_(hs, dZ, gU, None, shift_T=T)
    if xd is not None:
        linear_wgrad_(xd, dZd, gW, None)
        linear_wgrad_(hds, dZd, gU, None, shift_T=T)


def lstm_layer_tbwd(dH, dHd, tape, ttape, U, act: int, W=None):
    if isinstance(tape, FTape):
        heads = [a for a in (dH, dHd) if isinstance(a, OuterAdjoint)]
        if heads and all(a is None or (isinstance(a, OuterAdjoint) and a.w is heads[0].w and a.d.dtype == torch.float32)
                         for a in (dH, dHd)):
            dZ, dZd = _ops().lstmf_tbwd(None, None, tape.t, ttape.t, U, int(act), tape.B, tape.T,
                                        None if dH is None else dH.d.contiguous(),
                                        None if dHd is None else dHd.d.contiguous(), heads[0].w.reshape(-1).contiguous())
        else:
            dH, dHd = _mat(dH), _mat(dHd)
            dZ, dZd = _ops().lstmf_tbwd(None if dH is None else dH.contiguous(), None if dHd is None else dHd.contiguous(),
                                        tape.t, ttape.t, U, int(act), tape.B, tape.T)
        return (dZ, dZd) if W is None else (dZ, dZd, linear_dgrad(dZ, W), linear_dgrad(dZd, W))
    if isinstance(tape, torch.Tensor):
        heads = [a for a in (dH, dHd) if isinstance(a, OuterAdjoint)]
        Wk = W if _lstm2_dx_fused(W) else None
        if heads and all(a is None or (isinstance(a, OuterAdjoint) and a.w is heads[0].w)
                                       for a in (dH, dHd)):
            w = heads[0].w.reshape(-1).contiguous()
            dZ, dZd, dX, dXd = _ops().lstm2_tbwd(None, None, tape, ttape, U, int(act), Wk,
                                                 None if dH is None else dH.d.contiguous(),
                                                 None if dHd is None else dHd.d.contiguous(), w)
        else:
            dH, dHd = _mat(dH), _mat(dHd)
            dZ, dZd, dX, dXd = _ops().lstm2_tbwd(None if dH is None else dH.contiguous(), dHd.contiguous(), tape,
                                                 ttape, U, int(act), Wk)
        if W is not None and Wk is None:
            dX, dXd = linear_dgrad(dZ, W), linear_dgrad(dZd, W)
        return (dZ, dZd) if W is None else (dZ, dZd, dX, dXd)
    dH, dHd = _mat(dH), _mat(dHd)
    gates, cs = tape
    zds, cds = ttape
    if dH is None:
        dH = torch.zeros_like(dHd)
    dZ, dZd = lstm_seq_tbwd(dH, dHd, gates, cs, zds, cds, U, act)
    return (dZ, dZd) if W is None else (dZ, dZd, linear_dgrad(dZ, W), linear_dgrad(dZd, W))
```

do-you-really-need-to-pay-2-20-hedge-fund-strategy-replication-via-machine-learning_amd/ops/reference.py:

```python
from __future__ import annotations

import torch
import torch.nn.functional as F

ACT_CODES = {"linear": 0, None: 0, "sigmoid": 1, "tanh": 2, "leaky_relu": 3, "relu": 4}
LRELU_ALPHA = 0.2
LN_EPS = 1e-3
KERAS_EPS = 1e-7


def act_code(name) -> int:
    return ACT_CODES[name]


def apply_act(x: torch.Tensor, act) -> torch.Tensor:
    a = act_code(act) if not isinstance(act, int) else act
    if a == 0:
        return x
    if a == 1:
        return torch.sigmoid(x)
    if a == 2:
        return torch.tanh(x)
    if a == 3:
        return F.leaky_relu(x, LRELU_ALPHA)
# ... 96 lines not shown
    n = torch.sqrt(torch.sum(g.reshape(g.shape[0], -1) ** 2, dim=1))
    return torch.mean((1 - n) ** 2)


def gan_loss(p: torch.Tensor, split: int, la: float, lb: float, kind: int, acc=torch.float32):
    pf = p.reshape(-1).to(acc)
    n = pf.numel()
    y = torch.full_like(pf, lb)
    y[:split] = la
    inv = torch.full_like(pf, 1.0 / max(n - split, 1))
    inv[:split] = 1.0 / max(split, 1)
    if kind == 0:
        lo, g = y * pf, y * inv
    else:
        o = pf.clamp(KERAS_EPS, 1 - KERAS_EPS)
        lo = -(y * torch.log(o + KERAS_EPS) + (1 - y) * torch.log(1 - o + KERAS_EPS))
        inside = ((pf > KERAS_EPS) & (pf < 1 - KERAS_EPS)).to(acc)
        g = -(y / (o + KERAS_EPS) - (1 - y) / (1 - o + KERAS_EPS)) * inside * inv
    li = lo * inv
    out = torch.stack([li[:split].sum(), li[split:].sum()])
    return out, g.to(p.dtype).reshape(p.shape)


def gp_coef(g: torch.Tensor, weight: float):
    B = g.shape[0]
    gf = g.reshape(B, -1)
    n = torch.sqrt(torch.sum(gf * gf, dim=1))
    pen = torch.mean((1 - n) ** 2)
    scale = -(2.0 * weight / B) * (1 - n) / torch.clamp(n, min=1e-30)
    v = (gf * scale[:, None]).reshape(g.shape)
    return pen, v


def wdist_sorted(x: torch.Tensor, ref_sorted: torch.Tensor) -> torch.Tensor:
    xs = torch.sort(x.to(torch.float64), dim=0).values
    w = (xs - ref_sorted.to(torch.float64).t()).abs().mean(dim=0)
    return torch.cat([w, w.mean().reshape(1)])


def lstm_seq_fwd(zx: torch.Tensor, U: torch.Tensor, act: int, save: bool = True):
    B, T, G = zx.shape
    H = G // 4
    h = zx.new_zeros(B, H)
    c = zx.new_zeros(B, H)
    hs = zx.new_empty(B, T, H)
    gates = zx.new_empty(B, T, G) if save else None
    cs = zx.new_empty(B, T, H) if save else None
    for t in range(T):
        z = zx[:, t] + h @ U
        i = torch.sigmoid(z[:, :H])
        f = torch.sigmoid(z[:, H:2 * H])
        g = apply_act(z[:, 2 * H:3 * H], act)
        o = torch.sigmoid(z[:, 3 * H:])
        c = f * c + i * g
        h = o * apply_act(c, act)
        hs[:, t] = h
        if save:
            gates[:, t] = torch.cat([i, f, g, o], dim=1)
            cs[:, t] = c
    return hs, gates, cs


def lstm_seq_bwd(dh_seq: torch.Tensor, gates: torch.Tensor, cs: torch.Tensor, U: torch.Tensor, act: int):
    B, T, G = gates.shape
    H = G // 4
    dz_all = torch.empty_like(gates)
    dh = dh_seq.new_zeros(B, H)
    dc = dh_seq.new_zeros(B, H)
    Ut = U.t()
    for t in range(T - 1, -1, -1):
        i, f, g, o = gates[:, t].split(H, dim=1)
        c = cs[:, t]
        cp = cs[:, t - 1] if t > 0 else torch.zeros_like(c)
        ca = apply_act(c, act)
        dht = dh_seq[:, t] + dh
        do = dht * ca
        dct = dc + dht * o * act_dy(ca, act)
        di, dg, df = dct * g, dct * i, dct * cp
        dc = dct * f
        dz = torch.cat([di * i * (1 - i), df * f * (1 - f), dg * act_dy(g, act), do * o * (1 - o)], dim=1)
        dz_all[:, t] = dz
        dh = dz @ Ut
    return dz_all


def lstm_seq_tfwd(dzx: torch.Tensor, gates: torch.Tensor, cs: torch.Tensor, U: torch.Tensor, act: int):
    B, T, G = gates.shape
    H = G // 4
    hd = dzx.new_zeros(B, H)
    cd = dzx.new_zeros(B, H)
    hds = dzx.new_empty(B, T, H)
    zds = dzx.new_empty(B, T, G)
    cds = dzx.new_empty(B, T, H)
    for t in range(T):
        zd = dzx[:, t] + hd @ U
        i, f, g, o = gates[:, t].split(H, dim=1)
        c = cs[:, t]
        cp = cs[:, t - 1] if t > 0 else torch.zeros_like(c)
        idot = i * (1 - i) * zd[:, :H]
        fdot = f * (1 - f) * zd[:, H:2 * H]
        gdot = act_dy(g, act) * zd[:, 2 * H:3 * H]
        odot = o * (1 - o) * zd[:, 3 * H:]
        cd = fdot * cp + f * cd + idot * g + i * gdot
        ca = apply_act(c, act)
        hd = odot * ca + o * act_dy(ca, act) * cd
        hds[:, t] = hd
        zds[:, t] = zd
        cds[:, t] = cd
    return hds, zds, cds


def lstm_seq_tbwd(dh_seq, dhd_seq, gates, cs, zds, cds, U, act: int):
    B, T, G = gates.shape
    H = G // 4
    dZ = torch.empty_like(gates)
    dZd = torch.empty_like(gates)
    ah_n = gates.new_zeros(B, H)
    ahd_n = gates.new_zeros(B, H)
    ac_n = gates.new_zeros(B, H)
    acd_n = gates.new_zeros(B, H)
    Ut = U.t()
    for t in range(T - 1, -1, -1):
        i, f, g, o = gates[:, t].split(H, dim=1)
        c = cs[:, t]
        cd = cds[:, t]
        cp = cs[:, t - 1] if t > 0 else torch.zeros_like(c)
        cdp = cds[:, t - 1] if t > 0 else torch.zeros_like(c)
        zd = zds[:, t]
        zdi, zdf, zdg, zdo = zd.split(H, dim=1)
        si, sf, so = i * (1 - i), f * (1 - f), o * (1 - o)
        sg = act_dy(g, act)
        idot, fdot, gdot, odot = si * zdi, sf * zdf, sg * zdg, so * zdo
        ca = apply_act(c, act)
        d1 = act_dy(ca, act)
        d2 = act_d2y(ca, act)
        a_h = dh_seq[:, t] + ah_n
        a_hd = dhd_seq[:, t] + ahd_n
        a_od = a_hd * ca
        a_o = a_h * ca + a_hd * d1 * cd
        a_cd = acd_n + a_hd * o * d1
        a_c = ac_n + a_h * o * d1 + a_hd * (odot * d1 + o * d2 * cd)
        a_fd = a_cd * cp
        a_id = a_cd * g
        a_gd = a_cd * i
        a_f = a_c * cp + a_cd * cdp
        a_i = a_c * g + a_cd * gdot
        a_g = a_c * i + a_cd * idot
        ac_n = a_c * f + a_cd * fdot
        acd_n = a_cd * f
        s2i = si * (1 - 2 * i)
        s2f = sf * (1 - 2 * f)
        s2o = so * (1 - 2 * o)
        s2g = act_d2y(g, act)
        dzd = torch.cat([a_id * si, a_fd * sf, a_gd * sg, a_od * so], dim=1)
        dz = torch.cat([a_i * si + a_id * s2i * zdi, a_f * sf + a_fd * s2f * zdf,
                        a_g * sg + a_gd * s2g * zdg, a_o * so + a_od * s2o * zdo], dim=1)
        dZ[:, t] = dz
        dZd[:, t] = dzd
        ah_n = dz @ Ut
        ahd_n = dzd @ Ut
    return dZ, dZd


def shift_prev(h_seq: torch.Tensor) -> torch.Tensor:
    out = torch.zeros_like(h_seq)
    out[:, 1:] = h_seq[:, :-1]
    return out


def layer_norm_fwd(x: torch.Tensor, gamma, beta, eps: float = LN_EPS):
    mu = x.mean(dim=-1, keepdim=True)
    var = ((x - mu) ** 2).mean(dim=-1, keepdim=True)
    rstd = torch.rsqrt(var + eps)
    xhat = (x - mu) * rstd
    return xhat * gamma + beta, xhat, rstd


def layer_norm_bwd(dy: torch.Tensor, xhat: torch.Tensor, rstd: torch.Tensor, gamma):
    g = dy * gamma
    n = xhat.shape[-1]
    dx = rstd * (g - g.mean(dim=-1, keepdim=True) - xhat * (g * xhat).mean(dim=-1, keepdim=True))
    red = tuple(range(dy.dim() - 1))
    return dx, (dy * xhat).sum(dim=red), dy.sum(dim=red)


def layer_norm_tfwd(xd: torch.Tensor, xhat: torch.Tensor, rstd: torch.Tensor, gamma):
    m = (xhat * xd).mean(dim=-1, keepdim=True)
    return gamma * (rstd * (xd - xd.mean(dim=-1, keepdim=True) - xhat * m))


def layer_norm_tbwd(dy, dyd: torch.Tensor, xd: torch.Tensor, xhat: torch.Tensor, rstd: torch.Tensor, gamma):
    D = xhat.shape[-1]
    r = rstd
    mxd = xd.mean(dim=-1, keepdim=True)
    m = (xhat * xd).mean(dim=-1, keepdim=True)
    xhatd = r * (xd - mxd - xhat * m)
    h = dyd * gamma
    mh = h.mean(dim=-1, keepdim=True)
    S = (h * xhat).sum(dim=-1, keepdim=True)
    P = (h * xd).sum(dim=-1, keepdim=True)
    dxd = r * (h - mh - xhat * S / D)
    g = dy * gamma if dy is not None else torch.zeros_like(h)
    G = g - r * m * h - (r * S / D) * xd
    dx = r * (G - G.mean(dim=-1, keepdim=True) - xhat * (G * xhat).mean(dim=-1, keepdim=True)) \
        - r * r * xhat * (P - D * mxd * mh - m * S) / D
    red = tuple(range(dyd.dim() - 1))
    dgamma = (dyd * xhatd).sum(dim=red)
    dbeta = torch.zeros_like(dgamma)
    if dy is not None:
        dgamma = dgamma + (dy * xhat).sum(dim=red)
        dbeta = dy.sum(dim=red)
    return dx, dxd, dgamma, dbeta
```

do-you-really-need-to-pay-2-20-hedge-fund-strategy-replication-via-machine-learning_amd/train/gan_trainer.py:

```python
from __future__ import annotations

import os
import time
from dataclasses import dataclass, field

import numpy as np
import torch

from ..models import gan as zoo
from ..ops import functional as Fn
from ..utils.rng import DeviceRNG
from ..utils.trace import trange
from .optim import KerasOptimizer


@dataclass
class GANConfig:
    arch: str = "lstm"
    loss: str = "wgan_gp"
    window: int = 48
    features: int = 35
    batch_size: int = 32
    epochs: int = 5000
    n_critic: int | None = None
# ... 110 lines not shown
        return hook

    def _sync(self, model):
        if self.grad_sync is not None:
            with trange("allreduce"):
                if self.grad_sync.finish_() == 0:
                    self.grad_sync.all_reduce_(model.flat.grad)

    def _apply(self, model, clip=0.0):
        self._sync(model)
        with trange("optimizer"):
            self.opt.apply(model.flat, clip=clip)
            model.zero_grad()

    def _bce_step(self, x, label: float):
        C = self.critic
        p, tape = C.efwd(x, save=True)
        out, dp = Fn.gan_loss(p, p.numel(), label, label, 1)
        C.ebwd(tape, dp, hook=self._hook(C))
        self._apply(C)
        return out[0].to(self._acc)

    def _wgan_step(self, x, label: float, clip: float):
        C = self.critic
        s, tape = C.efwd(x, save=True)
        out, ds = Fn.gan_loss(s, s.numel(), label, label, 0)
        C.ebwd(tape, ds, hook=self._hook(C))
        self._apply(C, clip=clip)
        return out[0].to(self._acc)

    def _gp_step(self, real, noise, xrf=None, keep_gen_tape=False):
        dst = None if xrf is None else xrf[real.shape[0]:]
        with trange("critic/generate"):
            if keep_gen_tape:
                fake, gtape = self.generator.efwd(noise, save=True, out=dst)
            else:
                fake, gtape = self.generator.predict(noise, out=dst), None
            alpha = self.rng.uniform((real.shape[0],))
        out = self.critic_gp_grads(real, fake, alpha, xrf=xrf)
        self._apply(self.critic)
        return out, ((fake, gtape) if keep_gen_tape else None)

    def _gp_critic_steps_overlapped(self, B):
        cfg, G = self.cfg, self.generator
        side = self._side(1)
        cur = torch.cuda.current_stream(self.device)
        last = self.n_critic - 1

        def sample():
            with trange("critic/sample"):
                xrf = torch.empty((2 * B, cfg.window, cfg.features), dtype=self.dtype, device=self.device)
                real, noise = self._batch(B, out=xrf[:B])
            return xrf, real, noise

        def generate(noise, xrf, keep):
            with trange("critic/generate"):
                if keep:
                    return G.efwd(noise, save=True, out=xrf[B:])
                return G.predict(noise, out=xrf[B:]), None

        xrf, real, noise = sample()
        fake, gtape = generate(noise, xrf, self.reuse_gen_forward and last == 0)
        for k in range(self.n_critic):
            with trange("critic/generate"):
                alpha = self.rng.uniform((B,))
            if k < last:
                nxt = sample()
                side.wait_stream(cur)
                with torch.cuda.stream(side):
                    gnext = generate(nxt[2], nxt[0], self.reuse_gen_forward and k + 1 == last)
            self._d_acc = self.critic_gp_grads(real, fake, alpha, xrf=xrf)
            self._apply(self.critic)
            if k < last:
                cur.wait_stream(side)
                (xrf, real, noise), (fake, gtape) = nxt, gnext
        return noise, ((fake, gtape) if self.reuse_gen_forward else None)

    def critic_gp_grads(self, real, fake, alpha, xrf=None):
        C = self.critic
        xh = Fn.interpolate(real, fake, alpha)
        if xrf is None:
            xrf = torch.cat([real, fake], 0)
        side = self._side(0)
        if side is not None:
            cur = torch.cuda.current_stream(self.device)
            side.wait_stream(cur)
            with torch.cuda.stream(side), trange("critic/gp_input_grad"):
                sh, tape_h = C.efwd(xh, save=True, head_out=False)
                g = C.ebwd(tape_h, self._ones(sh), need_dx=True, wgrad=False)
                pen, v = Fn.gp_coef(g, self.gp_weight)
                sd, ttape = C.etfwd(tape_h, v.to(xh.dtype), head_out=False)
        hook = self._hook(C)
        with Fn.wgrad_on(self._wgrad_side(hook)):
            with trange("critic/w_terms"):
                n2 = xrf.shape[0] // 2
                hw = (n2, Fn.loss_grad_value(-1.0, n2, xrf.dtype), Fn.loss_grad_value(1.0, xrf.shape[0] - n2, xrf.dtype))
                s, tape = C.efwd(xrf, save=True, head_wgrad=hw)
                w, ds = Fn.gan_loss(s, s.numel() // 2, -1.0, 1.0, 0)
                C.ebwd(tape, ds)
            if side is not None:
                cur.wait_stream(side)
            if side is None:
                with trange("critic/gp_input_grad"):
                    sh, tape_h = C.efwd(xh, save=True, head_out=False)
                    g = C.ebwd(tape_h, self._ones(sh), need_dx=True, wgrad=False)
                    pack, v = Fn.gp_coef_pack(g, self.gp_weight, w)
                with trange("critic/gp_second_order"):
                    sd, ttape = C.etfwd(tape_h, v.to(xh.dtype), head_out=False)
            else:
                pack = Fn.gp_pack(pen, self.gp_weight, w)
            with trange("critic/gp_second_order"):
                C.etbwd(tape_h, ttape, None, self._ones(sd), hook=hook)
        return pack.to(self._acc)

    def _ones(self, like):
        key = (tuple(like.shape), like.dtype, like.device)
        t = self._ones_cache.get(key)
        if t is None:
            t = self._ones_cache[key] = torch.ones_like(like)
        return t

    def _generator_step(self, noise, gen=None):
        with trange("generator"):
            loss = self.generator_grads(noise, gen=gen)
        self._apply(self.generator)
        return loss

    def generator_grads(self, noise, gen=None):
        G, C = self.generator, self.critic
        fake, tg = gen if gen is not None else G.efwd(noise, save=True)
        s, tc = C.efwd(fake, save=True)
        if self.cfg.loss == "gan":
            out, ds = Fn.gan_loss(s, s.numel(), 1.0, 1.0, 1)
        else:
            out, ds = Fn.gan_loss(s, s.numel(), -1.0, -1.0, 0)
        loss = out[0].to(self._acc)
        dfake = C.ebwd(tc, ds, need_dx=True, wgrad=False)
        hook = self._hook(G)
        with Fn.wgrad_on(self._wgrad_side(hook)):
            G.ebwd(tg, dfake, hook=hook)
        return loss

    @torch.no_grad()
    def train_step(self):
        cfg, B = self.cfg, self.cfg.batch_size
        if self._fused is not None:
            self._fused.train_step()
        elif cfg.loss == "gan":
            real, noise = self._batch(B)
            fake = self.generator.predict(noise)
            lr_ = self._bce_step(real, 1.0)
            lf_ = self._bce_step(fake, 0.0)
            d = 0.5 * (lr_ + lf_)
            self._d_acc = torch.stack([d, lr_, lf_, torch.zeros_like(d)])
            noise2 = self.rng.normal((B, cfg.window, cfg.features), dtype=self.dtype)
            self._g_acc = self._generator_step(noise2).reshape(1)
        elif cfg.loss == "wgan":
            gen = None
            for k in range(self.n_critic):
                real, noise = self._batch(B)
                if self.reuse_gen_forward and k == self.n_critic - 1:
                    gen = self.generator.efwd(noise, save=True)
                    fake = gen[0]
                else:
                    fake = self.generator.predict(noise)
                lr_ = self._wgan_step(real, -1.0, 0.0)
                lf_ = self._wgan_step(fake, 1.0, self.clip)
                self._d_acc = torch.stack([0.5 * (lr_ + lf_), lr_, lf_, torch.zeros_like(lr_)])
            self._g_acc = self._generator_step(noise, gen=gen).reshape(1)
        elif self._side(1) is not None:
            noise, gen = self._gp_critic_steps_overlapped(B)
            self._g_acc = self._generator_step(noise, gen=gen).reshape(1)
        else:
            gen = None
            for k in range(self.n_critic):
                with trange("critic/sample"):
                    xrf = torch.empty((2 * B, cfg.window, cfg.features), dtype=self.dtype, device=self.device)
                    real, noise = self._batch(B, out=xrf[:B])
                self._d_acc, gen = self._gp_step(real, noise, xrf, keep_gen_tape=self.reuse_gen_forward and k == self.n_critic - 1)
            self._g_acc = self._generator_step(noise, gen=gen).reshape(1)
        self.iteration += 1

    def close(self) -> None:
        if self.grad_sync is not None:
            self.grad_sync.close()

    def losses(self) -> dict:
        d = self._d_acc.detach().float().cpu().numpy()
        return {"iteration": self.iteration, "d_loss": float(d[0]), "d_real": float(d[1]), "d_fake": float(d[2]),
                "gp": float(d[3]), "g_loss": float(self._g_acc.detach().float().cpu()[0])}

    def allreduce_floats_per_step(self) -> int:
        loss = self.cfg.loss
        updates = 2 if loss == "gan" else 2 * self.n_critic if loss == "wgan" else self.n_critic
        return updates * self.critic.flat.numel() + self.generator.flat.numel()
# ... 38 lines not shown
```

Baseline: 1.410 million seq/s.

## Reuse first-order BPTT adjoints in gradient-penalty second-order backward

The first-order input-gradient backward through the critic LSTM now optionally saves its per-step hidden adjoints (aH). A new single-output tangent-backward kernel (lstmf_tbwd1) then takes these saved adjoints instead of recomputing the first-order adjoint recurrence alongside the second-order one. The unneeded dXd dgrad is also skipped. This roughly halves the recurrent work in the GP second-order pass, at the cost of extra memory traffic to write and read aH and a larger code surface.

```diff
diff --git a/do-you-really-need-to-pay-2-20-hedge-fund-strategy-replication-via-machine-learning_amd/csrc/bindings.cpp b/do-you-really-need-to-pay-2-20-hedge-fund-strategy-replication-via-machine-learning_amd/csrc/bindings.cpp
--- a/do-you-really-need-to-pay-2-20-hedge-fund-strategy-replication-via-machine-learning_amd/csrc/bindings.cpp
+++ b/do-you-really-need-to-pay-2-20-hedge-fund-strategy-replication-via-machine-learning_amd/csrc/bindings.cpp
@@ -335,8 +335,10 @@
   }
 }
 
+bool lstmf_ahd_supported() { return hfrep::lstmf_ahd_supported(); }
+
 Tensor lstmf_bwd(optional<Tensor> dH, Tensor tape, Tensor U, int64_t act, int64_t B, int64_t Tn, optional<Tensor> hd,
-                 optional<Tensor> hw) {
+                 optional<Tensor> hw, optional<Tensor> ah_out) {
   CHECK_F32(tape);
   const int H = U.size(0);
   check_lstm_U(U, H);
@@ -345,6 +347,12 @@
   TORCH_CHECK(hd.has_value() == hw.has_value() && !(hd.has_value() && dH.has_value()),
               "lstmf_bwd: dH or the head factors (hd, hw)");
   check_head(hd, hw, tape, B, Tn * H);
+  if (ah_out.has_value()) {
+    CHECK_F32(*ah_out);
+    TORCH_CHECK(ah_out->numel() == B * Tn * H && ah_out->is_contiguous() && ah_out->device() == tape.device(),
+                "lstmf_bwd: ah_out must be a contiguous (B, T, H) fp32 tensor on the tape's device");
+    TORCH_CHECK(hfrep::lstmf_ahd_supported(), "lstmf_bwd: ah_out needs the split-recurrent BPTT (lstmf_ahd_supported)");
+  }
   GUARD(tape);
   Tensor dZ = out_empty({B, Tn, 4 * H}, tape.options());
   Tensor dHm;
@@ -357,8 +365,37 @@
   const float* dhp = dHm.defined() ? dHm.data_ptr<float>() : dH.has_value() ? dH->data_ptr<float>() : nullptr;
   const bool ok = hfrep::launch_lstmf_bwd(dhp, tape.data_ptr<float>(), U.data_ptr<float>(), dZ.data_ptr<float>(), B, Tn,
                                           H, (int)act, cur_stream(tape), head ? hd->data_ptr<float>() : nullptr,
-                                          head ? hw->data_ptr<float>() : nullptr);
+                                          head ? hw->data_ptr<float>() : nullptr,
+                                          ah_out.has_value() ? ah_out->data_ptr<float>() : nullptr);
   TORCH_CHECK(ok, "lstmf_bwd: unsupported H / act");
+  return dZ;
+}
+
+Tensor lstmf_tbwd1(optional<Tensor> dH, Tensor aH, Tensor tape, Tensor ttape, Tensor U, int64_t act, int64_t B,
+                   int64_t Tn, optional<Tensor> hd, optional<Tensor> hw) {
+  CHECK_F32(tape); CHECK_F32(ttape); CHECK_F32(aH);
+  const int H = U.size(0);
+  check_lstm_U(U, H);
+  TORCH_CHECK(tape.numel() == (int64_t)hfrep::lstmf_tape_elems(B, Tn) && ttape.numel() == tape.numel(), "tape size");
+  TORCH_CHECK(aH.numel() == B * Tn * H && aH.is_contiguous() && aH.device() == tape.device(),
+              "lstmf_tbwd1: aH must be a contiguous (B, T, H) fp32 tensor on the tape's device");
+  if (dH.has_value()) {
+    CHECK_F32(*dH);
+    TORCH_CHECK(dH->numel() == B * Tn * H && dH->is_contiguous() && dH->device() == tape.device(),
+                "lstmf_tbwd1: adjoint shape");
+  }
+  const bool head = hw.has_value();
+  TORCH_CHECK(!head || !dH.has_value(), "lstmf_tbwd1: the adjoint dH or head factors, not both");
+  TORCH_CHECK(head || !hd.has_value(), "lstmf_tbwd1: hd needs hw");
+  check_head(hd, hw, tape, B, Tn * H);
+  GUARD(tape);
+  Tensor dZ = out_empty({B, Tn, 4 * H}, tape.options());
+  const bool ok = hfrep::launch_lstmf_tbwd1(dH.has_value() ? dH->data_ptr<float>() : nullptr, aH.data_ptr<float>(),
+                                            tape.data_ptr<float>(), ttape.data_ptr<float>(), U.data_ptr<float>(),
+                                            dZ.data_ptr<float>(), B, Tn, H, (int)act, cur_stream(tape),
+                                            head && hd.has_value() ? hd->data_ptr<float>() : nullptr,
+                                            head ? hw->data_ptr<float>() : nullptr);
+  TORCH_CHECK(ok, "lstmf_tbwd1: unsupported H / act");
   return dZ;
 }
 
@@ -974,7 +1011,11 @@
   m.def("lstmf_fwd(Tensor x, Tensor W, Tensor? b, Tensor U, int act, bool save) -> (Tensor, Tensor)");
   m.def("linear_head_cs(Tensor x, Tensor W, Tensor? b, int split, float wa, float wb, Tensor(a!) gW, Tensor(b!)? gb) -> Tensor");
   m.def("linear_head_cs_supported(int K) -> bool", &linear_head_cs_supported);
-  m.def("lstmf_bwd(Tensor? dH, Tensor tape, Tensor U, int act, int B, int T, Tensor? hd=None, Tensor? hw=None) -> Tensor");
+  m.def("lstmf_bwd(Tensor? dH, Tensor tape, Tensor U, int act, int B, int T, Tensor? hd=None, Tensor? hw=None, "
+        "Tensor(a!)? ah_out=None) -> Tensor");
+  m.def("lstmf_ahd_supported() -> bool", &lstmf_ahd_supported);
+  m.def("lstmf_tbwd1(Tensor? dH, Tensor aH, Tensor tape, Tensor ttape, Tensor U, int act, int B, int T, Tensor? hd=None, "
+        "Tensor? hw=None) -> Tensor");
   m.def("lstmf_tbwd(Tensor? dH, Tensor? dHd, Tensor tape, Tensor ttape, Tensor U, int act, int B, int T, Tensor? hd=None, "
         "Tensor? hdd=None, Tensor? hw=None) -> (Tensor, Tensor)");
   m.def("lstmf_tfwd(Tensor xd, Tensor W, Tensor U, Tensor tape, int act) -> (Tensor, Tensor)");
@@ -1036,6 +1077,7 @@
   m.impl("linear_head_cs", &linear_head_cs);
   m.impl("lstmf_bwd", &lstmf_bwd);
   m.impl("lstmf_tbwd", &lstmf_tbwd);
+  m.impl("lstmf_tbwd1", &lstmf_tbwd1);
   m.impl("lstmf_dgrad", &lstmf_dgrad);
   m.impl("fp3_split", &fp3_split);
   m.impl("fp3_join", &fp3_join);
diff --git a/do-you-really-need-to-pay-2-20-hedge-fund-strategy-replication-via-machine-learning_amd/csrc/kernels.h b/do-you-really-need-to-pay-2-20-hedge-fund-strategy-replication-via-machine-learning_amd/csrc/kernels.h
--- a/do-you-really-need-to-pay-2-20-hedge-fund-strategy-replication-via-machine-learning_amd/csrc/kernels.h
+++ b/do-you-really-need-to-pay-2-20-hedge-fund-strategy-replication-via-machine-learning_amd/csrc/kernels.h
@@ -37,8 +37,12 @@
 bool launch_lstmf_tfwd(const float* xd, const float* W, const float* U, const float* tape, float* hds, float* ttape,
                        int B, int Tn, int K, int H, int act, hipStream_t s);
 bool launch_lstmf_bwd(const float* dH, const float* tape, const float* U, float* dZ, int B, int Tn, int H, int act,
-                      hipStream_t s, const float* hd = nullptr, const float* hw = nullptr);
+                      hipStream_t s, const float* hd = nullptr, const float* hw = nullptr, float* aH = nullptr);
 bool lstmf_head_supported();
+bool lstmf_ahd_supported();
+bool launch_lstmf_tbwd1(const float* dH, const float* aH, const float* tape, const float* ttape, const float* U, float* dZ,
+                        int B, int Tn, int H, int act, hipStream_t s, const float* hd = nullptr,
+                        const float* hw = nullptr);
 bool launch_lstmf_tbwd(const float* dH, const float* dHd, const float* tape, const float* ttape, const float* U, float* dZ,
                        float* dZd, int B, int Tn, int H, int act, hipStream_t s, const float* hd = nullptr,
                        const float* hdd = nullptr, const float* hw = nullptr);
diff --git a/do-you-really-need-to-pay-2-20-hedge-fund-strategy-replication-via-machine-learning_amd/csrc/lstm_f32.hip b/do-you-really-need-to-pay-2-20-hedge-fund-strategy-replication-via-machine-learning_amd/csrc/lstm_f32.hip
--- a/do-you-really-need-to-pay-2-20-hedge-fund-strategy-replication-via-machine-learning_amd/csrc/lstm_f32.hip
+++ b/do-you-really-need-to-pay-2-20-hedge-fund-strategy-replication-via-machine-learning_amd/csrc/lstm_f32.hip
@@ -739,6 +739,201 @@
         half_b(I1{});
         __builtin_amdgcn_sched_barrier(0);
         load_half(I0{}, t > 0 ? t - 1 : 0, t > 0);
+        lds_barrier();
+      }
+      __syncthreads();
+    }
+  }
+}
+
+#ifndef HFREP_TBWD1_CELLGROUP
+#define HFREP_TBWD1_CELLGROUP 2
+#endif
+#ifndef HFREP_TBWD1_EARLYLOAD
+#define HFREP_TBWD1_EARLYLOAD 1
+#endif
+template <int ACT, bool HEAD = false>
+__global__ void __launch_bounds__(512, 1)
+lstmf_tbwd1_kernel(const float* __restrict__ dH, const float* __restrict__ aH, const float* __restrict__ tape,
+                   const float* __restrict__ ttape, const float* __restrict__ U, float* __restrict__ dZ, int B, int Tn,
+                   const float* __restrict__ hd, const float* __restrict__ hw) {
+  extern __shared__ __attribute__((aligned(16))) float fsm[];
+  float* zt = fsm;
+  float* ht = zt + 32 * BZ_LR;
+  float* trash = ht + 32 * BH_LR;
+  const int tid = threadIdx.x, lane = tid & 63;
+  const int wv = __builtin_amdgcn_readfirstlane(tid >> 6);
+  const int w = wv & 3;
+  const int q = lane & 3, g = lane >> 4, j4 = (lane & 15) >> 2, c16 = lane & 15;
+  const int nrb = (B + 31) / 32;
+  if (wv < 4) {
+    float ut[2][FH];
+#pragma unroll
+    for (int e = 0; e < 2; ++e) {
+      const int j = 16 * (2 * w + e) + c16;
+      const bool ok = j < FH;
+#pragma unroll
+      for (int k = 0; k < FH; ++k) {
+        const float v = U[(ok ? j : 0) * FG + g * FH + k];
+        ut[e][k] = ok ? v : 0.f;
+      }
+    }
+    auto half_a = [&](auto MA_) {
+      constexpr int M = decltype(MA_)::value;
+      f32x4 acc[2] = {f32x4{0.f, 0.f, 0.f, 0.f}, f32x4{0.f, 0.f, 0.f, 0.f}};
+      const float* ar = zt + (16 * M + c16) * BZ_LR + g * BZ_KQ;
+#pragma unroll
+      for (int jj = 0; jj < FH / 4; ++jj) {
+        const f32x4 a4 = *reinterpret_cast<const f32x4*>(ar + 4 * jj);
+#pragma unroll
+        for (int s = 0; s < 4; ++s) {
+          acc[0] = mma4(a4[s], ut[0][4 * jj + s], acc[0]);
+          acc[1] = mma4(a4[s], ut[1][4 * jj + s], acc[1]);
+        }
+        if ((jj & 1) == 1) __builtin_amdgcn_sched_barrier(0);
+      }
+#pragma unroll
+      for (int e = 0; e < 2; ++e) {
+        const int col = 16 * (2 * w + e) + c16;
+        if (2 * w + e < 7) {
+#pragma unroll
+          for (int i = 0; i < 4; ++i) ht[(16 * M + 4 * g + i) * BH_LR + col] = acc[e][i];
+        }
+      }
+    };
+    const int srr = tid / 100, sch = tid - 100 * srr, sqq = sch / 25, sc = sch - 25 * sqq;
+    const int slo = (srr & 1) * BZ_LR + sqq * BZ_KQ + 4 * sc;
+    const int sgo = tid < 200 ? (srr * Tn * FG + sqq * FH + 4 * sc) * 4 : kOOB;
+    using I0 = std::integral_constant<int, 0>;
+    using I1 = std::integral_constant<int, 1>;
+    for (int rb = blockIdx.x; rb < nrb; rb += gridDim.x) {
+      const int row0 = rb * 32;
+      const rsrc_t rz = ftile_rsrc(dZ, row0, B, Tn, FG);
+      const int nr = min(32, B - row0);
+      auto store_half = [&](auto M_, int ts) {
+        constexpr int M = decltype(M_)::value;
+#pragma unroll
+        for (int k = 8 * M; k < 8 * M + 8; ++k) {
+          const f32x4 v = *reinterpret_cast<const f32x4*>(zt + slo + 2 * k * BZ_LR);
+          st16(v, rz, 2 * k + srr < nr, sgo, (2 * k * Tn + ts) * FG * 4);
+          if (k & 1) __builtin_amdgcn_sched_barrier(0);
+        }
+        __builtin_amdgcn_sched_barrier(0);
+      };
+      for (int i = tid; i < 32 * (BZ_LR + BH_LR); i += 512) zt[i] = 0.f;
+      __syncthreads();
+      for (int t = Tn - 1; t >= 0; --t) {
+        if (t < Tn - 1) store_half(I1{}, t + 1);
+        half_a(I1{});
+        lds_barrier();
+        store_half(I0{}, t);
+        half_a(I0{});
+        lds_barrier();
+      }
+      store_half(I1{}, 0);
+      __syncthreads();
+    }
+  } else {
+    const int ub = FUW * w + j4;
+    const int hr = (4 * g + q) * BH_LR + ub, zw = (4 * g + q) * BZ_LR + ub;
+    const int tl = ftape_lane(w, lane), tcl = ftape_cell(w, lane);
+    for (int rb = blockIdx.x; rb < nrb; rb += gridDim.x) {
+      const int row0 = rb * 32;
+      const rsrc_t rdh = ftile_rsrc(dH, row0, B, Tn, FH), rah = ftile_rsrc(aH, row0, B, Tn, FH);
+      const rsrc_t rt = ftape_rsrc(tape, rb, nrb, Tn), rtt = ftape_rsrc(ttape, rb, nrb, Tn);
+      int vp1[2];
+#pragma unroll
+      for (int m = 0; m < 2; ++m) vp1[m] = ((16 * m + 4 * g + q) * Tn * FH + ub) * 4;
+      float hdv[2] = {0.f, 0.f};
+      const rsrc_t rhw = make_rsrc(hw, HEAD ? Tn * FH * 4 : 0);
+      if constexpr (HEAD) {
+#pragma unroll
+        for (int m = 0; m < 2; ++m) {
+          const int r = row0 + 16 * m + 4 * g + q;
+          hdv[m] = (hd && r < B) ? hd[r] : 0.f;
+        }
+      }
+      const int hvo = ub * 4;
+      float tc[2][FNT], tcd[2][FNT], acn[2][FNT], acdn[2][FNT];
+      f32x4 tg[FNT], tz[FNT];
+      float tcp[FNT], tcdp[FNT], tdh[FNT], tah[FNT];
+      auto load_cell = [&](auto M_, int n, int tt, bool on) {
+        constexpr int m = decltype(M_)::value;
+        const int tp = tt > 0 ? tt - 1 : 0;
+        const bool tok = on && !(w == 3 && n >= 4);
+        const int sg = tt * FT_STEP * 4 + ftape_slot(m, n), sc = tp * FT_STEP * 4 + ftape_slot(m, n);
+        const int sd = tt * FH * 4 + 16 * n;
+        tg[n] = __builtin_bit_cast(f32x4, __builtin_amdgcn_raw_buffer_load_b128(rt, tok ? tl : kOOB, sg, 0));
+        tz[n] = __builtin_bit_cast(f32x4, __builtin_amdgcn_raw_buffer_load_b128(rtt, tok ? tl : kOOB, sg, 0));
+        tcp[n] = ld1(rt, (tok && tt > 0) ? tcl : kOOB, sc);
+        tcdp[n] = ld1(rtt, (tok && tt > 0) ? tcl : kOOB, sc);
+        if constexpr (HEAD) tdh[n] = hdv[m] * ld1(rhw, tok ? hvo : kOOB, sd);
+        else tdh[n] = ld1(rdh, tok ? vp1[m] : kOOB, sd);
+        tah[n] = ld1(rah, tok ? vp1[m] : kOOB, sd);
+      };
+      auto load_half = [&](auto M_, int tt, bool on) {
+#pragma unroll
+        for (int n = 0; n < FNT; ++n) load_cell(M_, n, tt, on);
+      };
+#pragma unroll
+      for (int m = 0; m < 2; ++m)
+#pragma unroll
+        for (int n = 0; n < FNT; ++n) {
+          const bool tok = !(w == 3 && n >= 4);
+          const int oc = tcl + (Tn - 1) * FT_STEP * 4 + ftape_slot(m, n);
+          acn[m][n] = 0.f;
+          acdn[m][n] = 0.f;
+          tc[m][n] = ld1(rt, tok ? oc : kOOB, 0);
+          tcd[m][n] = ld1(rtt, tok ? oc : kOOB, 0);
+        }
+      load_half(std::integral_constant<int, 0>{}, Tn - 1, true);
+      for (int i = tid; i < 32 * (BZ_LR + BH_LR); i += 512) zt[i] = 0.f;
+      __syncthreads();
+      auto half_b = [&](auto M_, auto MN_, int tn, bool non) {
+        constexpr int m = decltype(M_)::value;
+#pragma unroll
+        for (int n = 0; n < FNT; ++n) {
+          const bool tok = !(w == 3 && n >= 4);
+          const float i_ = tg[n][0], f_ = tg[n][1], g_ = tg[n][2], o_ = tg[n][3];
+          const float zdi = tz[n][0], zdf = tz[n][1], zdg = tz[n][2], zdo = tz[n][3];
+          const float c = tc[m][n], cd = tcd[m][n], cp = tcp[n], cdp = tcdp[n];
+          const float si = i_ * (1.f - i_), sf = f_ * (1.f - f_), so = o_ * (1.f - o_), sg = act_dy(ACT, g_);
+          const float idot = si * zdi, fdot = sf * zdf, gdot = sg * zdg, odot = so * zdo;
+          const float ca = act_f(ACT, c), d1 = act_dy(ACT, ca), d2 = act_d2y(ACT, ca);
+          const float a_h = tdh[n] + ht[hr + 16 * m * BH_LR + 4 * n], a_hd = tah[n];
+          const float a_od = a_hd * ca;
+          const float a_o = a_h * ca + a_hd * d1 * cd;
+          const float a_cd = acdn[m][n] + a_hd * o_ * d1;
+          const float a_c = acn[m][n] + a_h * o_ * d1 + a_hd * (odot * d1 + o_ * d2 * cd);
+          const float a_fd = a_cd * cp, a_id = a_cd * g_, a_gd = a_cd * i_;
+          const float a_f = a_c * cp + a_cd * cdp;
+          const float a_i = a_c * g_ + a_cd * gdot;
+          const float a_g = a_c * i_ + a_cd * idot;
+          acn[m][n] = tok ? a_c * f_ + a_cd * fdot : 0.f;
+          acdn[m][n] = tok ? a_cd * f_ : 0.f;
+          const float s2i = si * (1.f - 2.f * i_), s2f = sf * (1.f - 2.f * f_), s2o = so * (1.f - 2.f * o_);
+          const float s2g = act_d2y(ACT, g_);
+          float z4[4];
+          z4[0] = a_i * si + a_id * s2i * zdi;
+          z4[1] = a_f * sf + a_fd * s2f * zdf;
+          z4[2] = a_g * sg + a_gd * s2g * zdg;
+          z4[3] = a_o * so + a_od * s2o * zdo;
+          float* zp = tok ? zt + zw + 16 * m * BZ_LR + 4 * n : trash;
+#pragma unroll
+          for (int k = 0; k < 4; ++k) zp[k * BZ_KQ] = z4[k];
+          tc[m][n] = cp;
+          tcd[m][n] = cdp;
+          if constexpr (HFREP_TBWD1_EARLYLOAD) load_cell(MN_, n, tn, non);
+          if ((n + 1) % HFREP_TBWD1_CELLGROUP == 0 || n == FNT - 1) __builtin_amdgcn_sched_barrier(0);
+        }
+        if constexpr (!HFREP_TBWD1_EARLYLOAD) load_half(MN_, tn, non);
+      };
+      using I0 = std::integral_constant<int, 0>;
+      using I1 = std::integral_constant<int, 1>;
+      for (int t = Tn - 1; t >= 0; --t) {
+        half_b(I0{}, I1{}, t, true);
+        lds_barrier();
+        half_b(I1{}, I0{}, t > 0 ? t - 1 : 0, t > 0);
         lds_barrier();
       }
       __syncthreads();
@@ -1711,10 +1906,11 @@
 constexpr int BS_LZ = 432;
 constexpr int BS_PL = 32 * BS_LZ * 2;
 
-template <int ACT, bool HEAD = false>
+template <int ACT, bool HEAD = false, bool AHD = false>
 __global__ void __launch_bounds__(256, 1)
 lstmf_bwds_kernel(const float* __restrict__ dH, const float* __restrict__ tape, const float* __restrict__ U,
-                  float* __restrict__ dZ, int B, int Tn, const float* __restrict__ hd, const float* __restrict__ hw) {
+                  float* __restrict__ dZ, int B, int Tn, const float* __restrict__ hd, const float* __restrict__ hw,
+                  float* __restrict__ aH) {
   extern __shared__ __attribute__((aligned(16))) float fsm[];
   float* zt = fsm;
   float* ht = zt + 32 * BZ_LR;
@@ -1763,6 +1959,7 @@
     const int row0 = rb * 32;
     const rsrc_t rdh = ftile_rsrc(dH, row0, B, Tn, FH), rt = ftape_rsrc(tape, rb, nrb, Tn);
     const rsrc_t rz = ftile_rsrc(dZ, row0, B, Tn, FG);
+    const rsrc_t rah = ftile_rsrc(AHD ? aH : nullptr, row0, B, Tn, FH);
     const int nr = min(32, B - row0);
     int vp1[2];
 #pragma unroll
@@ -1840,6 +2037,7 @@
                                max(tp - 1, 0) * FT_STEP * 4 + ftape_slot(0, n), tp * FH * 4 + 16 * n, tok && t > 0,
                                tp > 0, hdv[0], rhw, hvo);
       }
+      if constexpr (AHD) st1(dht, rah, tok ? vp1[m] : kOOB, t * FH * 4 + 16 * n);
     };
     auto phase = [&](auto MA_, int t) {
       constexpr int MA = decltype(MA_)::value;
@@ -2233,7 +2431,7 @@
 }
 template <int ACT>
 void bwdf_launch(const float* dH, const float* tape, const float* U, float* dZ, int B, int Tn, hipStream_t s,
-                 const float* hd, const float* hw) {
+                 const float* hd, const float* hw, float* aH) {
   const int ver = bwdf_impl().load(std::memory_order_relaxed);
   const int nrb = (B + 31) / 32, cus = device_cu_count();
   const size_t sm = (size_t)(32 * BZ_LR + 32 * BH_LR + 4 * BZ_KQ) * 4;
@@ -2241,12 +2439,18 @@
     auto go = [&](auto k) {
       allow_lds(reinterpret_cast<const void*>(k));
       hipLaunchKernelGGL(k, dim3(nrb < cus ? nrb : cus), dim3(256), sm + 16 + 3 * BS_PL, s, dH, tape, U, dZ, B, Tn, hd,
-                         hw);
+                         hw, aH);
     };
-    if (hd) go(lstmf_bwds_kernel<ACT, true>);
-    else go(lstmf_bwds_kernel<ACT, false>);
+    if (aH) {
+      if (hd) go(lstmf_bwds_kernel<ACT, true, true>);
+      else go(lstmf_bwds_kernel<ACT, false, true>);
+    } else {
+      if (hd) go(lstmf_bwds_kernel<ACT, true>);
+      else go(lstmf_bwds_kernel<ACT, false>);
+    }
     return;
   }
+  if (aH) throw std::runtime_error("lstmf_bwd: the exact-fp32 BPTT does not store the h adjoints (lstmf_ahd_supported)");
   if (hd) throw std::runtime_error("lstmf_bwd: the exact-fp32 BPTT takes a materialised dH (lstmf_head_supported)");
   auto k = lstmf_bwdp_kernel<ACT>;
   allow_lds(reinterpret_cast<const void*>(k));
@@ -2255,13 +2459,14 @@
 static_assert((32 * BZ_LR + 32 * BH_LR + 4 * BZ_KQ) * 4 + 16 + 3 * BS_PL <= F_LDS_MAX, "split BPTT LDS");
 int set_lstmf_bwd_impl(int v) { return bwdf_impl().exchange(v); }
 bool lstmf_head_supported() { return bwdf_impl().load(std::memory_order_relaxed) != 2; }
+bool lstmf_ahd_supported() { return bwdf_impl().load(std::memory_order_relaxed) != 2; }
 bool launch_lstmf_bwd(const float* dH, const float* tape, const float* U, float* dZ, int B, int Tn, int H, int act,
-                      hipStream_t s, const float* hd, const float* hw) {
+                      hipStream_t s, const float* hd, const float* hw, float* aH) {
   if (H != FH || B <= 0 || Tn <= 0) return false;
   switch (act) {
-    case ACT_LINEAR: bwdf_launch<ACT_LINEAR>(dH, tape, U, dZ, B, Tn, s, hd, hw); return true;
-    case ACT_SIGMOID: bwdf_launch<ACT_SIGMOID>(dH, tape, U, dZ, B, Tn, s, hd, hw); return true;
-    case ACT_TANH: bwdf_launch<ACT_TANH>(dH, tape, U, dZ, B, Tn, s, hd, hw); return true;
+    case ACT_LINEAR: bwdf_launch<ACT_LINEAR>(dH, tape, U, dZ, B, Tn, s, hd, hw, aH); return true;
+    case ACT_SIGMOID: bwdf_launch<ACT_SIGMOID>(dH, tape, U, dZ, B, Tn, s, hd, hw, aH); return true;
+    case ACT_TANH: bwdf_launch<ACT_TANH>(dH, tape, U, dZ, B, Tn, s, hd, hw, aH); return true;
     default: return false;
   }
 }
@@ -2288,6 +2493,29 @@
     case ACT_LINEAR: tbwdf_launch<ACT_LINEAR>(dH, dHd, tape, ttape, U, dZ, dZd, B, Tn, s, hd, hdd, hw); return true;
     case ACT_SIGMOID: tbwdf_launch<ACT_SIGMOID>(dH, dHd, tape, ttape, U, dZ, dZd, B, Tn, s, hd, hdd, hw); return true;
     case ACT_TANH: tbwdf_launch<ACT_TANH>(dH, dHd, tape, ttape, U, dZ, dZd, B, Tn, s, hd, hdd, hw); return true;
+    default: return false;
+  }
+}
+template <int ACT>
+void tbwd1f_launch(const float* dH, const float* aH, const float* tape, const float* ttape, const float* U, float* dZ,
+                   int B, int Tn, hipStream_t s, const float* hd, const float* hw) {
+  const int cus = device_cu_count();
+  const size_t sm = (size_t)(32 * BZ_LR + 32 * BH_LR + 4 * BZ_KQ) * 4;
+  const int nrb = (B + 31) / 32;
+  auto go = [&](auto k) {
+    allow_lds(reinterpret_cast<const void*>(k));
+    hipLaunchKernelGGL(k, dim3(nrb < cus ? nrb : cus), dim3(512), sm, s, dH, aH, tape, ttape, U, dZ, B, Tn, hd, hw);
+  };
+  if (hw) go(lstmf_tbwd1_kernel<ACT, true>);
+  else go(lstmf_tbwd1_kernel<ACT, false>);
+}
+bool launch_lstmf_tbwd1(const float* dH, const float* aH, const float* tape, const float* ttape, const float* U, float* dZ,
+                        int B, int Tn, int H, int act, hipStream_t s, const float* hd, const float* hw) {
+  if (H != FH || B <= 0 || Tn <= 0 || !aH) return false;
+  switch (act) {
+    case ACT_LINEAR: tbwd1f_launch<ACT_LINEAR>(dH, aH, tape, ttape, U, dZ, B, Tn, s, hd, hw); return true;
+    case ACT_SIGMOID: tbwd1f_launch<ACT_SIGMOID>(dH, aH, tape, ttape, U, dZ, B, Tn, s, hd, hw); return true;
+    case ACT_TANH: tbwd1f_launch<ACT_TANH>(dH, aH, tape, ttape, U, dZ, B, Tn, s, hd, hw); return true;
     default: return false;
   }
 }
diff --git a/do-you-really-need-to-pay-2-20-hedge-fund-strategy-replication-via-machine-learning_amd/models/layers.py b/do-you-really-need-to-pay-2-20-hedge-fund-strategy-replication-via-machine-learning_amd/models/layers.py
--- a/do-you-really-need-to-pay-2-20-hedge-fund-strategy-replication-via-machine-learning_amd/models/layers.py
+++ b/do-you-really-need-to-pay-2-20-hedge-fund-strategy-replication-via-machine-learning_amd/models/layers.py
@@ -68,7 +68,7 @@
     def etfwd(self, ctx, xd):
         raise NotImplementedError
 
-    def etbwd(self, ctx, tctx, dy, dyd, need_dx: bool):
+    def etbwd(self, ctx, tctx, dy, dyd, need_dx: bool, need_dxd: bool = True):
         raise NotImplementedError
 
     def w(self, name):
@@ -128,7 +128,7 @@
         yd = Fn.act_backward(zd, ctx["y"], self.act_code)
         return yd, {"xd": xd, "zd": zd}
 
-    def etbwd(self, ctx, tctx, dy, dyd, need_dx):
+    def etbwd(self, ctx, tctx, dy, dyd, need_dx, need_dxd=True):
         dzd = Fn.act_backward(dyd, ctx["y"], self.act_code)
         zero_dz = dy is None and self.act_code in (0, 3, 4)
         if not zero_dz:
@@ -137,7 +137,7 @@
         Fn.run_wgrad(Fn.linear_wgrad_, tctx["xd"], dzd, self.g("kernel"), None)
         if not need_dx:
             return None, None
-        return (None if zero_dz else self._dgrad(dz)), self._dgrad(dzd)
+        return (None if zero_dz else self._dgrad(dz)), (self._dgrad(dzd) if need_dxd else None)
 
 
 class LSTM(Layer):
@@ -168,9 +168,19 @@
                                      save)
         return hs, ({"x": x, "hs": hs, "tape": tape} if save else None)
 
-    def ebwd(self, ctx, dy, need_dx, wgrad=True):
+    def ebwd(self, ctx, dy, need_dx, wgrad=True, keep=None):
         U = self.p("recurrent_kernel")
         dx = None
+        if keep is not None:
+            got = Fn.lstm_layer_bwd_keep(dy, ctx["tape"], U, self.act_code, W=self.p("kernel") if need_dx else None)
+            if got is not None:
+                dZ, dx, keep["ahd"] = got
+                keep["dZ"] = dZ
+                keep["dy"] = None
+                if wgrad:
+                    Fn.run_wgrad(Fn.lstm_wgrad_, ctx["x"], ctx["hs"], dZ, self.g("kernel"), self.g("recurrent_kernel"),
+                                 self.g("bias"))
+                return dx
         if need_dx:
             dZ, dx = Fn.lstm_layer_bwd(dy, ctx["tape"], U, self.act_code, W=self.p("kernel"), need_dz=wgrad)
         else:
@@ -183,12 +193,18 @@
         hds, ttape = Fn.lstm_layer_tfwd(xd, self.p("kernel"), ctx["tape"], self.p("recurrent_kernel"), self.act_code)
         return hds, {"xd": xd, "hds": hds, "ttape": ttape}
 
-    def etbwd(self, ctx, tctx, dy, dyd, need_dx):
+    def etbwd(self, ctx, tctx, dy, dyd, need_dx, need_dxd=True, brec=None):
         U = self.p("recurrent_kernel")
         dx = dxd = None
-        if need_dx:
+        if brec is not None and "ahd" in brec:
+            dZd, ahd = brec.pop("dZ"), brec.pop("ahd")
+            dZ = Fn.lstm_layer_tbwd1(dy, ahd, ctx["tape"], tctx["ttape"], U, self.act_code)
+            del ahd
+            if need_dx:
+                dx = Fn.linear_dgrad(dZ, self.p("kernel"))
+        elif need_dx:
             dZ, dZd, dx, dxd = Fn.lstm_layer_tbwd(dy, dyd, ctx["tape"], tctx["ttape"], U, self.act_code,
-                                                  W=self.p("kernel"))
+                                                  W=self.p("kernel"), need_dxd=need_dxd)
         else:
             dZ, dZd = Fn.lstm_layer_tbwd(dy, dyd, ctx["tape"], tctx["ttape"], U, self.act_code)
         Fn.run_wgrad(Fn.lstm_wgrad_, ctx["x"], ctx["hs"], dZ, self.g("kernel"), self.g("recurrent_kernel"), self.g("bias"),
@@ -223,7 +239,7 @@
     def etfwd(self, ctx, xd):
         return Fn.layer_norm_tfwd(xd, ctx["xhat"], ctx["rstd"], self.p("gamma")), {"xd": xd}
 
-    def etbwd(self, ctx, tctx, dy, dyd, need_dx):
+    def etbwd(self, ctx, tctx, dy, dyd, need_dx, need_dxd=True):
         return Fn.layer_norm_tbwd_(dy, dyd, tctx["xd"], ctx["xhat"], ctx["rstd"], self.p("gamma"), self.g("gamma"),
                                    self.g("beta"), need_dx)
 
@@ -251,11 +267,11 @@
     def etfwd(self, ctx, xd):
         return Fn.act_backward(xd, ctx["y"], 3), {}
 
-    def etbwd(self, ctx, tctx, dy, dyd, need_dx):
+    def etbwd(self, ctx, tctx, dy, dyd, need_dx, need_dxd=True):
         if not need_dx:
             return None, None
         dx = Fn.act_backward(dy, ctx["y"], 3) if dy is not None else None
-        return dx, Fn.act_backward(dyd, ctx["y"], 3)
+        return dx, (Fn.act_backward(dyd, ctx["y"], 3) if need_dxd else None)
 
 
 class Flatten(Layer):
@@ -278,7 +294,7 @@
     def etfwd(self, ctx, xd):
         return xd.reshape(xd.shape[0], -1), {}
 
-    def etbwd(self, ctx, tctx, dy, dyd, need_dx):
+    def etbwd(self, ctx, tctx, dy, dyd, need_dx, need_dxd=True):
         if not need_dx:
             return None, None
         return (dy.reshape(ctx["shape"]) if dy is not None else None), dyd.reshape(ctx["shape"])
@@ -325,7 +341,7 @@
         zd = Fn.linear(cols_d, self.p("kernel").reshape(-1, self.filters), None, 0)
         return Fn.act_backward(zd, ctx["y"], self.act_code), {"cols_d": cols_d, "zd": zd}
 
-    def etbwd(self, ctx, tctx, dy, dyd, need_dx):
+    def etbwd(self, ctx, tctx, dy, dyd, need_dx, need_dxd=True):
         Wk = self.p("kernel").reshape(-1, self.filters)
         gk = self.g("kernel").reshape(-1, self.filters)
         if dy is None:
@@ -337,7 +353,7 @@
         if not need_dx:
             return None, None
         return (Fn.col2im_causal(Fn.linear_dgrad(dz, Wk), self.k, self.dil, self.cin),
-                Fn.col2im_causal(Fn.linear_dgrad(dzd, Wk), self.k, self.dil, self.cin))
+                Fn.col2im_causal(Fn.linear_dgrad(dzd, Wk), self.k, self.dil, self.cin) if need_dxd else None)
 
 
 def _init_tensor(spec: ParamSpec, gen, layer: Layer) -> torch.Tensor:
@@ -494,14 +510,21 @@
             return dy.materialize()
         return dy
 
-    def ebwd(self, tape, dy, need_dx: bool = False, wgrad: bool = True, hook=None):
+    def ebwd(self, tape, dy, need_dx: bool = False, wgrad: bool = True, hook=None, keep: bool = False):
+        btape = [None] * len(self.layers)
         for i in range(len(self.layers) - 1, -1, -1):
             need = need_dx or i > 0
             layer = self.layers[i]
-            dy = layer.ebwd(tape[i], self._adj(layer, dy), need, wgrad)
+            dy = self._adj(layer, dy)
+            if keep:
+                btape[i] = {"dy": dy}
+                dy = layer.ebwd(tape[i], dy, need, wgrad, keep=btape[i]) if isinstance(layer, LSTM) else \
+                    layer.ebwd(tape[i], dy, need, wgrad)
+            else:
+                dy = layer.ebwd(tape[i], dy, need, wgrad)
             if hook is not None:
                 hook(i)
-        return Fn._mat(dy)
+        return (Fn._mat(dy), btape) if keep else Fn._mat(dy)
 
     def etfwd(self, tape, xd, head_out: bool = True):
         skip_head = not head_out and self._head_skippable()
@@ -515,11 +538,17 @@
             ttape.append(tctx)
         return xd, ttape
 
-    def etbwd(self, tape, ttape, dy, dyd, need_dx: bool = False, hook=None):
+    def etbwd(self, tape, ttape, dy, dyd, need_dx: bool = False, hook=None, btape=None):
         for i in range(len(self.layers) - 1, -1, -1):
             need = need_dx or i > 0
             layer = self.layers[i]
-            dy, dyd = layer.etbwd(tape[i], ttape[i], self._adj(layer, dy), self._adj(layer, dyd), need)
+            if btape is not None:
+                rec = btape[i]
+                kw = {"brec": rec} if isinstance(layer, LSTM) else {}
+                dy, _ = layer.etbwd(tape[i], ttape[i], self._adj(layer, dy), rec["dy"], need, need_dxd=False, **kw)
+                dyd = btape[i] = rec = None
+            else:
+                dy, dyd = layer.etbwd(tape[i], ttape[i], self._adj(layer, dy), self._adj(layer, dyd), need)
             if hook is not None:
                 hook(i)
         return Fn._mat(dy), Fn._mat(dyd)
diff --git a/do-you-really-need-to-pay-2-20-hedge-fund-strategy-replication-via-machine-learning_amd/ops/functional.py b/do-you-really-need-to-pay-2-20-hedge-fund-strategy-replication-via-machine-learning_amd/ops/functional.py
--- a/do-you-really-need-to-pay-2-20-hedge-fund-strategy-replication-via-machine-learning_amd/ops/functional.py
+++ b/do-you-really-need-to-pay-2-20-hedge-fund-strategy-replication-via-machine-learning_amd/ops/functional.py
@@ -346,6 +346,42 @@
     dH = _mat(dH)
     gates, cs = tape
     dZ = lstm_seq_bwd(dH, gates, cs, U, act)
+    return dZ if W is None else (dZ, linear_dgrad(dZ, W))
+
+
+def lstm_layer_bwd_keep(dH, tape, U, act: int, W=None):
+    if isinstance(tape, FTape):
+        if not _ops().lstmf_ahd_supported():
+            return None
+        ah = torch.empty((tape.B, tape.T, U.shape[0]), dtype=torch.float32, device=tape.t.device)
+        if isinstance(dH, OuterAdjoint) and dH.d.dtype == torch.float32:
+            dZ = _ops().lstmf_bwd(None, tape.t, U, int(act), tape.B, tape.T, dH.d.contiguous(),
+                                  dH.w.reshape(-1).contiguous(), ah)
+        else:
+            dH = _mat(dH)
+            dZ = _ops().lstmf_bwd(None if dH is None else dH.contiguous(), tape.t, U, int(act), tape.B, tape.T, None,
+                                  None, ah)
+        return dZ, (None if W is None else linear_dgrad(dZ, W)), ah
+    if isinstance(tape, torch.Tensor) or _nat(tape[0]):
+        return None
+    gates, cs = tape
+    dZ, ah = R.lstm_seq_bwd_ahd(_mat(dH), gates, cs, U.to(gates.dtype), act)
+    return dZ, (None if W is None else linear_dgrad(dZ, W)), ah
+
+
+def lstm_layer_tbwd1(dH, a_hd, tape, ttape, U, act: int, W=None):
+    if isinstance(tape, FTape):
+        if isinstance(dH, OuterAdjoint) and dH.d.dtype == torch.float32:
+            dZ = _ops().lstmf_tbwd1(None, a_hd, tape.t, ttape.t, U, int(act), tape.B, tape.T, dH.d.contiguous(),
+                                    dH.w.reshape(-1).contiguous())
+        else:
+            dH = _mat(dH)
+            dZ = _ops().lstmf_tbwd1(None if dH is None else dH.contiguous(), a_hd, tape.t, ttape.t, U, int(act), tape.B,
+                                    tape.T)
+    else:
+        gates, cs = tape
+        zds, cds = ttape
+        dZ = R.lstm_seq_tbwd_ahd(_mat(dH), a_hd, gates, cs, zds, cds, U.to(gates.dtype), act)
     return dZ if W is None else (dZ, linear_dgrad(dZ, W))
 
 
@@ -378,7 +414,7 @@
         linear_wgrad_(hds, dZd, gU, None, shift_T=T)
 
 
-def lstm_layer_tbwd(dH, dHd, tape, ttape, U, act: int, W=None):
+def lstm_layer_tbwd(dH, dHd, tape, ttape, U, act: int, W=None, need_dxd: bool = True):
     if isinstance(tape, FTape):
         heads = [a for a in (dH, dHd) if isinstance(a, OuterAdjoint)]
         if heads and all(a is None or (isinstance(a, OuterAdjoint) and a.w is heads[0].w and a.d.dtype == torch.float32)
@@ -390,7 +426,7 @@
             dH, dHd = _mat(dH), _mat(dHd)
             dZ, dZd = _ops().lstmf_tbwd(None if dH is None else dH.contiguous(), None if dHd is None else dHd.contiguous(),
                                         tape.t, ttape.t, U, int(act), tape.B, tape.T)
-        return (dZ, dZd) if W is None else (dZ, dZd, linear_dgrad(dZ, W), linear_dgrad(dZd, W))
+        return (dZ, dZd) if W is None else (dZ, dZd, linear_dgrad(dZ, W), linear_dgrad(dZd, W) if need_dxd else None)
     if isinstance(tape, torch.Tensor):
         heads = [a for a in (dH, dHd) if isinstance(a, OuterAdjoint)]
         Wk = W if _lstm2_dx_fused(W) else None
@@ -405,7 +441,7 @@
             dZ, dZd, dX, dXd = _ops().lstm2_tbwd(None if dH is None else dH.contiguous(), dHd.contiguous(), tape,
                                                  ttape, U, int(act), Wk)
         if W is not None and Wk is None:
-            dX, dXd = linear_dgrad(dZ, W), linear_dgrad(dZd, W)
+            dX, dXd = linear_dgrad(dZ, W), linear_dgrad(dZd, W) if need_dxd else None
         return (dZ, dZd) if W is None else (dZ, dZd, dX, dXd)
     dH, dHd = _mat(dH), _mat(dHd)
     gates, cs = tape
@@ -413,4 +449,4 @@
     if dH is None:
         dH = torch.zeros_like(dHd)
     dZ, dZd = lstm_seq_tbwd(dH, dHd, gates, cs, zds, cds, U, act)
-    return (dZ, dZd) if W is None else (dZ, dZd, linear_dgrad(dZ, W), linear_dgrad(dZd, W))
+    return (dZ, dZd) if W is None else (dZ, dZd, linear_dgrad(dZ, W), linear_dgrad(dZd, W) if need_dxd else None)
diff --git a/do-you-really-need-to-pay-2-20-hedge-fund-strategy-replication-via-machine-learning_amd/ops/reference.py b/do-you-really-need-to-pay-2-20-hedge-fund-strategy-replication-via-machine-learning_amd/ops/reference.py
--- a/do-you-really-need-to-pay-2-20-hedge-fund-strategy-replication-via-machine-learning_amd/ops/reference.py
+++ b/do-you-really-need-to-pay-2-20-hedge-fund-strategy-replication-via-machine-learning_amd/ops/reference.py
@@ -202,6 +202,31 @@
         dz_all[:, t] = dz
         dh = dz @ Ut
     return dz_all
+
+
+def lstm_seq_bwd_ahd(dh_seq: torch.Tensor, gates: torch.Tensor, cs: torch.Tensor, U: torch.Tensor, act: int):
+    B, T, G = gates.shape
+    H = G // 4
+    dz_all = torch.empty_like(gates)
+    ah_all = torch.empty_like(cs)
+    dh = dh_seq.new_zeros(B, H)
+    dc = dh_seq.new_zeros(B, H)
+    Ut = U.t()
+    for t in range(T - 1, -1, -1):
+        i, f, g, o = gates[:, t].split(H, dim=1)
+        c = cs[:, t]
+        cp = cs[:, t - 1] if t > 0 else torch.zeros_like(c)
+        ca = apply_act(c, act)
+        dht = dh_seq[:, t] + dh
+        ah_all[:, t] = dht
+        do = dht * ca
+        dct = dc + dht * o * act_dy(ca, act)
+        di, dg, df = dct * g, dct * i, dct * cp
+        dc = dct * f
+        dz = torch.cat([di * i * (1 - i), df * f * (1 - f), dg * act_dy(g, act), do * o * (1 - o)], dim=1)
+        dz_all[:, t] = dz
+        dh = dz @ Ut
+    return dz_all, ah_all
 
 
 def lstm_seq_tfwd(dzx: torch.Tensor, gates: torch.Tensor, cs: torch.Tensor, U: torch.Tensor, act: int):
@@ -282,6 +307,46 @@
     return dZ, dZd
 
 
+def lstm_seq_tbwd_ahd(dh_seq, ahd_seq, gates, cs, zds, cds, U, act: int):
+    B, T, G = gates.shape
+    H = G // 4
+    dZ = torch.empty_like(gates)
+    ah_n = gates.new_zeros(B, H)
+    ac_n = gates.new_zeros(B, H)
+    acd_n = gates.new_zeros(B, H)
+    Ut = U.t()
+    for t in range(T - 1, -1, -1):
+        i, f, g, o = gates[:, t].split(H, dim=1)
+        c = cs[:, t]
+        cd = cds[:, t]
+        cp = cs[:, t - 1] if t > 0 else torch.zeros_like(c)
+        cdp = cds[:, t - 1] if t > 0 else torch.zeros_like(c)
+        zdi, zdf, zdg, zdo = zds[:, t].split(H, dim=1)
+        si, sf, so = i * (1 - i), f * (1 - f), o * (1 - o)
+        sg = act_dy(g, act)
+        idot, fdot, gdot, odot = si * zdi, sf * zdf, sg * zdg, so * zdo
+        ca = apply_act(c, act)
+        d1 = act_dy(ca, act)
+        d2 = act_d2y(ca, act)
+        a_h = ah_n if dh_seq is None else dh_seq[:, t] + ah_n
+        a_hd = ahd_seq[:, t]
+        a_od = a_hd * ca
+        a_o = a_h * ca + a_hd * d1 * cd
+        a_cd = acd_n + a_hd * o * d1
+        a_c = ac_n + a_h * o * d1 + a_hd * (odot * d1 + o * d2 * cd)
+        a_fd, a_id, a_gd = a_cd * cp, a_cd * g, a_cd * i
+        a_f = a_c * cp + a_cd * cdp
+        a_i = a_c * g + a_cd * gdot
+        a_g = a_c * i + a_cd * idot
+        ac_n = a_c * f + a_cd * fdot
+        acd_n = a_cd * f
+        dz = torch.cat([a_i * si + a_id * si * (1 - 2 * i) * zdi, a_f * sf + a_fd * sf * (1 - 2 * f) * zdf,
+                        a_g * sg + a_gd * act_d2y(g, act) * zdg, a_o * so + a_od * so * (1 - 2 * o) * zdo], dim=1)
+        dZ[:, t] = dz
+        ah_n = dz @ Ut
+    return dZ
+
+
 def shift_prev(h_seq: torch.Tensor) -> torch.Tensor:
     out = torch.zeros_like(h_seq)
     out[:, 1:] = h_seq[:, :-1]
diff --git a/do-you-really-need-to-pay-2-20-hedge-fund-strategy-replication-via-machine-learning_amd/train/gan_trainer.py b/do-you-really-need-to-pay-2-20-hedge-fund-strategy-replication-via-machine-learning_amd/train/gan_trainer.py
--- a/do-you-really-need-to-pay-2-20-hedge-fund-strategy-replication-via-machine-learning_amd/train/gan_trainer.py
+++ b/do-you-really-need-to-pay-2-20-hedge-fund-strategy-replication-via-machine-learning_amd/train/gan_trainer.py
@@ -216,12 +216,27 @@
         if xrf is None:
             xrf = torch.cat([real, fake], 0)
         side = self._side(0)
+        reuse = os.environ.get("HFREP_GP_REUSE", "1") != "0"
+        btape = None
+
+        def input_grad(sh, tape_h):
+            ones = self._ones(sh)
+            if not reuse:
+                return C.ebwd(tape_h, ones, need_dx=True, wgrad=False), None
+            return C.ebwd(tape_h, ones, need_dx=True, wgrad=False, keep=True)
+
+        def second_order(sd, tape_h, ttape, btape, hook):
+            ones = self._ones(sd)
+            if btape is not None:
+                assert ones is btape[-1]["dy"], "adjoint reuse needs the same ones seed on both passes"
+            C.etbwd(tape_h, ttape, None, ones, hook=hook, btape=btape)
+
         if side is not None:
             cur = torch.cuda.current_stream(self.device)
             side.wait_stream(cur)
             with torch.cuda.stream(side), trange("critic/gp_input_grad"):
                 sh, tape_h = C.efwd(xh, save=True, head_out=False)
-                g = C.ebwd(tape_h, self._ones(sh), need_dx=True, wgrad=False)
+                g, btape = input_grad(sh, tape_h)
                 pen, v = Fn.gp_coef(g, self.gp_weight)
                 sd, ttape = C.etfwd(tape_h, v.to(xh.dtype), head_out=False)
         hook = self._hook(C)
@@ -232,19 +247,20 @@
                 s, tape = C.efwd(xrf, save=True, head_wgrad=hw)
                 w, ds = Fn.gan_loss(s, s.numel() // 2, -1.0, 1.0, 0)
                 C.ebwd(tape, ds)
+                del tape, s, ds
             if side is not None:
                 cur.wait_stream(side)
             if side is None:
                 with trange("critic/gp_input_grad"):
                     sh, tape_h = C.efwd(xh, save=True, head_out=False)
-                    g = C.ebwd(tape_h, self._ones(sh), need_dx=True, wgrad=False)
+                    g, btape = input_grad(sh, tape_h)
                     pack, v = Fn.gp_coef_pack(g, self.gp_weight, w)
                 with trange("critic/gp_second_order"):
                     sd, ttape = C.etfwd(tape_h, v.to(xh.dtype), head_out=False)
             else:
                 pack = Fn.gp_pack(pen, self.gp_weight, w)
             with trange("critic/gp_second_order"):
-                C.etbwd(tape_h, ttape, None, self._ones(sd), hook=hook)
+                second_order(sd, tape_h, ttape, btape, hook)
         return pack.to(self._acc)
 
     def _ones(self, like):
```

Result: faster. 1.483 million seq/s, median of 6 (+5.2%).
